# qingqing-zijin/LEAD-YOLO

Hardware: AMD Instinct MI355X
Metric: images/sec (640x640) fwd+bwd (higher is better)
Workload: dtype bf16; 1 GPU; lead-yolo-s bs=64/gpu 3x640x640 bf16 full train step: uint8 batch -> train-mode forward (batch-statistics BN), ComputeLoss, HIP backward, clip 10, SGD-nesterov 3 groups, ModelEMA update (BASELINE.json configs[2]); random-init weights; global_batch=64, parallelism=dp1 (single GPU, no collective), world_size=1

## Files before the change

### include/lead_yolo_hip.h

```cpp
#ifndef LEAD_YOLO_HIP_H
#define LEAD_YOLO_HIP_H
#ifdef __cplusplus
extern "C" {
#endif

enum { LY_F32 = 0, LY_BF16 = 1 };
int ly_abi_version(void);
const char* ly_last_error(void);

int ly_mlpblock_fwd(const void* x , void* y , int n_img, int H, int W, int C, const void* wp, const void* w1,
                    const void* w2, const float* bn_scale, const float* bn_shift, double* stats, int dtype, void* stream);
int ly_mlpblock_pconv(const void* x , void* z , int n_img, int H, int W, int C, const void* wp, int dtype, void* stream);
int ly_mlpblock_bwd_ok(int C, int dtype);
long ly_mlpblock_bwd_slab_floats(int C);
int ly_mlpblock_bwd(const void* x , const void* dy , void* g , int n_img, int H, int W, int C, const void* wp, const void* w1,
                    const void* w2t, const void* w1t, const float* a, const float* b, const float* alpha, const float* kappa, const float* lambda,
                    double* stats, float* slab, long slab_floats, float* dw1, float* dw2, int pass, int dtype, void* stream);
int ly_mlpblock_bwd_dx_ok(int C, int W, int dtype);
int ly_mlpblock_bwd_dx(const void* g , const void* dy , const void* x , void* dx , int n_img, int H, int W, int C, const void* wpt,
                       float* slab, long slab_floats, float* dwp, int lddw, int dw_ts, int dw_cs, int dtype, void* stream);
int ly_mlpblock_hidden_tiles(int C);

enum { LY_ACT_NONE_ = 0, LY_ACT_RELU_ = 1, LY_ACT_SILU_ = 2 };
enum { LY_GATHER_ROWS = 0,
       LY_GATHER_UP2 = 1,
       LY_GATHER_PATCH = 2,
       LY_GATHER_PATCH_NCHW = 3,
       LY_GATHER_PATCH_NCHW_U8 = 4,
       LY_GATHER_PATCH_NCHW_BF16 = 5,
       LY_GATHER_PATCH_NCHW_F16 = 6    };
enum { LY_PRO_NONE = 0,
       LY_PRO_GATE = 1,
       LY_PRO_AFFINE_RELU_CA = 2      };

typedef struct LyGemmParams {
  long M;
  int H, W;
  int K, N;
  const void* a0; int lda0; int k0;
  const void* a1; int lda1;
  int gather;
  int Hin, Win, Cin, ks, pk;
  int pro;
  const float* g_h; const float* g_w;
  const void* res; int ldres;
  const float* p_scale; const float* p_shift; const float* p_ca;
  const void* wp;
  const float* e_scale; const float* e_shift;
  const float* rowscale;
  int act;
  void* out; int ldo;
  double* stats;
  int dtype;
  int scat_ks, scat_c;
  const void* eadd; int ldeadd;
} LyGemmParams;

int ly_gemm_fwd(const LyGemmParams* p, void* stream);


typedef struct LyConv3Params {
  long M; int H, W;
  int Cin, N;
  int TH, TW;
  const void* x; int ldx;
  const void* wp;
  const float* e_scale; const float* e_shift;
  int act;
  void* out; int ldo;
  double* stats;
  int dtype;
} LyConv3Params;

int ly_conv3x3_fwd(const LyConv3Params* p, void* stream);


int ly_pool_hw(const void* x , int ldx, int n_img, int H, int W, int C, float* pool, int dtype, void* stream);
int ly_coordatt_mlp(const float* pool, int n_img, int H, int W, int C, int mip, const float* w1, const float* b1,
                    const float* sc, const float* sh, const float* wh, const float* bh, const float* ww, const float* bw, float* a_h,
                    float* a_w, void* stream);
int ly_coordatt_mlp_bwd(const float* pool, int n_img, int H, int W, int C, int mip, const float* w1, const float* b1,
                        const float* mean, const float* invstd, const float* gamma, const float* beta, const float* wh,
                        const float* ww, const float* a_h, const float* a_w, const float* da_h, const float* da_w, float* ws,
                        double* sums , float* dpool, float* dw1, float* dgamma, float* dbeta, float* dwh, float* dbh, float* dww,
                        float* dbw, int grads_f64 , void* stream);

int ly_coordatt_gate(const void* x , int ldx, int n_img, int H, int W, int C, const float* a_h, const float* a_w,
                     const void* res , int ldres, void* out , int ldo, int dtype, void* stream);

int ly_se_fwd(const void* x , int ldx, int n_img, int HW, int C, const float* wa, const float* wb, int R, float* part,
              int slices, float* ca, int dtype, void* stream);
int ly_rfcbam_stats(const void* x , int ldx, int n_img, int H, int W, int C, int k, int s, const float* wg,
                    const float* a1, const float* b1, int TH, int TW, float* mm, float* part, int slices, int dtype, void* stream);
int ly_colsum(const void* x , int ldx, int n_img, int HW, int C, float* part, int slices, int dtype, void* stream);
int ly_rfcbam_mid(const float* part, int slices, int C, int HW, const float* wa, const float* wb, int R, float* ca, int n_img,
                  const float* mm, int HK, int WK, const float* w18, float* rfa, void* stream);
int ly_rfa_map(const float* mm, int n_img, int HK, int WK, const float* w, float* rfa, void* stream);

typedef struct LyRfcbam3Params {
  int n_img, H, W, C;
  int Ho, Wo, N, s;
  int TH, TW;
  const void* x; int ldx;
  const float* wg;
  const float* ca;
  const float* rfa;
  const void* wp;
  const float* e_scale; const float* e_shift;
  void* out; int ldo;
  double* stats;
  int linear;
  int dtype;
} LyRfcbam3Params;
int ly_rfcbam3_fwd(const LyRfcbam3Params* p, void* stream);

int ly_rf3c_stats(const void* x , int ldx, int n_img, int H, int W, int C, int s, const float* wq, int raw, int TH, int TW, float* mm,
                  float* part, int slices, int dtype, void* stream);
int ly_rf3c_fwd(const LyRfcbam3Params* p, const float* wq, int raw, void* stream);

int ly_rf3m_stats(const void* x , int ldx, int n_img, int H, int W, int C, int s, const void* wst, int TH, int TW, float* mm, float* part,
                  int slices, void* stream);
int ly_rf3m_fwd(const LyRfcbam3Params* p, void* stream);

typedef struct LyRf3cBwdParams {
  int n_img, H, W, C;
  int Ho, Wo, O, s;
  int TH, TW;
  const void* x; int ldx;
  const void* du; int lddu;
  const float* wq;
  const void* wct;
  const float* ca;
  const float* rfa;
  const float* mm;
  const float* d_mm;
  const float* coef;
  float* d_rfa_part; float* d_ca;
  float* sums;
  float* dwg;
  void* dx; int lddx;
  const float* dgap; float dgap_scale;
  float* dwc_part; int ng;
  int dtype;
} LyRf3cBwdParams;
int ly_rf3c_bwd(const LyRf3cBwdParams* p, int pass, void* stream);
int ly_rf3c_wgrad(const LyRf3cBwdParams* p, void* stream);


int ly_sppf_pool(const void* x , int ldx, int n_img, int H, int W, int C, int k, void* out , int ldo, int dtype, void* stream);
int ly_detect_tail(const void* y , int ldy, int n_img, int H, int W, int na, int no, const float* anchors, float stride,
                   float* p, float* z, long zrows, long zoff, int dtype, void* stream);
int ly_detect_level(const void* x , int ldx, int n_img, int H, int W, int K, const void* wp, int nat, const float* bias, int na, int no,
                    const float* anchors, float stride, float* p, float* z, long zrows, long zoff, int dtype, void* stream);
int ly_detect_level_ok(int K, int na, int no, int dtype);
int ly_detect_level_aug(const void* x , int ldx, int n_img, int H, int W, int K, const void* wp, int nat, const float* bias, int na, int no,
                        const float* anchors, float stride, float* p, float* z, long zrows, long zoff, float dscale, int dflip, float img_w,
                        int dtype, void* stream);
int ly_detect_tail_aug(const void* y , int ldy, int n_img, int H, int W, int na, int no, const float* anchors, float stride,
                       float* p, float* z, long zrows, long zoff, float dscale, int dflip, float img_w, int dtype, void* stream);

enum { LY_F16 = 2 };
#define LY_SCALE_IMG_MAX 4
typedef struct LyScaleImgSpec {
  void* out;
  int Hs, Ws;
  int Ho, Wo;
  int flip;
} LyScaleImgSpec;
int ly_scale_img(const void* x , int n_img, int C, int H, int W, const LyScaleImgSpec* specs, int nspec, float pad, int dtype, void* stream);

typedef struct LyMosaicTile {
  long off;
  int h, w;
  int x1a, y1a, x2a, y2a;
  int x1b, y1b;
  int lab, nlab;
  int src;
  int unused;
  double padw, padh;
} LyMosaicTile;
typedef struct LyMosaicImage {
  LyMosaicTile tile[4];
  double m[6];
  float minv[6];
  double scale;
  int mosaic;
  int flipud, fliplr;
  int unused;
  const unsigned char* lut;
} LyMosaicImage;
int ly_mosaic_img(const unsigned char* bank, const LyMosaicImage* imgs, int n_img, int s, unsigned char* out, void* stream);
int ly_mosaic_labels(const double* labels, const LyMosaicImage* imgs, int n_img, int s, int max_labels, float* targets, long cap, void* stream);
typedef struct LyMixup {
  int partner;
  int unused;
  double r;
} LyMixup;
int ly_mosaic_mix_img(const unsigned char* bank, const LyMosaicImage* imgs, const LyMixup* mix, int n_img, int n_entry, int s, unsigned char* out,
                      void* stream);
int ly_mosaic_mix_labels(const double* labels, const LyMosaicImage* imgs, const LyMixup* mix, int n_img, int n_entry, int s, int max_labels,
                         float* targets, long cap, void* stream);
int ly_detect_head_bwd(const float* dp, int n_img, int H, int W, int na, int no, void* du , int ldu, float* dbias,
                       int dbias_f64 , int dtype, void* stream);


int ly_chan_moments(const void* x , int ldx, long rows, int C, double* mom , int dtype, void* stream);
int ly_coordatt_conv1_stats(const float* pool, long positions, int C, int mip, const float* w1, const float* b1,
                            double* stats , void* stream);
int ly_sum_rows_f64(const double* src, int R, int C, double* dst, void* stream);

int ly_rfcbam_tap_moments(const void* x , int ldx, int n_img, int H, int W, int C, int s, double* mom , int dtype, void* stream);
int ly_rfcbam_gen_prepare(const double* mom, int C, int k, const float* gen_w, const float* gamma, const float* beta, float eps,
                          float momentum, double count, float* running_mean, float* running_var, long* nbt, float* out8, float* a1,
                          float* wq_stats, float* wq_main, float* wq_c , int mom_stripes , void* stream);

int ly_nms_candidates(const float* pred, int bs, int N, int no, float conf_thres, unsigned long long class_mask, float* score, float* det,
                      void* stream);
int ly_nms_candidates_ml(const float* pred, int bs, int N, int no, float conf_thres, unsigned long long class_mask, float* score, float* det,
                         void* stream);
int ly_nms_greedy(const float* det, const long* order, const float* sorted_score, int bs, int N, float iou_thres, float max_wh, int max_det,
                  int max_nms, int* keep, int* count, void* stream);

#define LY_VAL_MAX_LABELS 512
int ly_val_match(const float* dets, const int* counts, int bs, int max_det, const float* targets, long nt, int W, int H, const float* shapes,
                 const float* levels, int single_cls, int nc, const int* cursor, int capacity, int row_width, void* correct, float* conf,
                 float* cls, int* match_label, float* match_iou, int* n_det, int* nt_class, int* overflow, void* stream);
int ly_val_advance(int* cursor, int bs, void* stream);
int ly_val_confusion(const float* dets, const int* counts, int bs, int max_det, const float* targets, long nt, int W, int H,
                     const float* shapes, float conf_thres, float iou_thres, int single_cls, int nc, int* matrix, int* flags, void* stream);

typedef struct LyLetterboxImage {
  const unsigned char* src;
  unsigned char* dst;
  int h0, w0;
  int H, W;
  int nh, nw;
  int top, left;
} LyLetterboxImage;
enum { LY_LB_CHW_RGB = 0, LY_LB_HWC_BGR = 1 };
int ly_letterbox_u8(const LyLetterboxImage* imgs, int n_img, int maxH, int maxW, int layout, void* stream);
int ly_scale_boxes(const float* dets, const int* counts, int bs, int max_det, const float* shapes, int round_boxes, float* out,
                   void* stream);


int ly_bnact_fwd(const void* u , int ldu, long rows, int C, const float* a, const float* b, int act, void* y , int ldy, int dtype, void* stream);
int ly_bnact_bwd_reduce(const void* dy , int lddy, const void* u , int ldu, long rows, int C, const float* a, const float* b,
                        int act, double* sums , int dtype, void* stream);
int ly_bnact_bwd_apply(const void* dy , int lddy, const void* u , int ldu, long rows, int C, const float* a, const float* b,
                       int act, const float* alpha, const float* kappa, const float* lambda, void* du , int lddu, int dtype, void* stream);
int ly_bnact_bwd_reduce_pair(const void* dy1 , int lddy1, const void* dy2 , int lddy2, int csplit, const void* u , int ldu, long rows, int C,
                             const float* a, const float* b, int act, double* sums1, double* sums2, int dtype, void* stream);
int ly_bnact_bwd_apply_pair(const void* dy1 , int lddy1, const void* dy2 , int lddy2, int csplit, const void* u , int ldu, long rows, int C,
                            const float* a, const float* b, int act, const float* alpha, const float* kappa, const float* lambda, void* du , int lddu,
                            int dtype, void* stream);

typedef struct LyWgradParams {
  long M;
  int H, W;
  int N;
  const void* du; int lddu;
  const void* x; int ldx;
  int Hin, Win, Cin;
  int ks, stride, pad;
  int nchw, up2;
  float* dw; int lddw;
  int dtype;
  int dw_ts, dw_cs, n_valid, c_valid;
  const float* x_scale; const float* x_shift;
  float* ws; long ws_floats;
} LyWgradParams;
int ly_wgrad(const LyWgradParams* p, void* stream);
int ly_wgrad_group(const LyWgradParams* arr, int n, void* stream);
int ly_tune_wgrad3(int on);

int ly_up2_bwd(const void* d , int ldd, int n_img, int Hs, int Ws, int C, void* out , int ldo, int dtype, void* stream);
int ly_unpatch(const void* g , int n_img, int Ho, int Wo, int C, int ks, void* dx , int dtype, void* stream);
int ly_sum_rows(const float* src, long R, long C, long ld, float* dst, int accumulate, void* stream);
int ly_patch4_rows_u8(const unsigned char* img, int n_img, int C, int H, int W, void* rows , int dtype, void* stream);
int ly_patch4_wgrad_u8(const unsigned char* img, int n_img, int C, int H, int W, const void* du , int lddu, int N, float scale, float* slab,
                       long slab_floats, float* dw , int dtype, void* stream);

int ly_coordatt_gate_bwd(const void* dout , int ldd, const void* x , int ldx, int n_img, int H, int W, int C, const float* a_h,
                         const float* a_w, void* dx , int lddx, float* da_h, float* da_w, int bands, int slabs, int dtype, void* stream);
int ly_pool_hw_bwd(const float* gp, int n_img, int H, int W, int C, void* dx , int lddx, int accumulate, int dtype, void* stream);
int ly_maxpool_arg(const void* x , int ldx, int n_img, int H, int W, int C, int k, unsigned char* arg, int lda, int dtype, void* stream);
int ly_maxpool_gather(const unsigned char* arg, int lda, const float* d_up, int ldu, const void* d_own, int ldd, int own_dtype, int n_img, int H,
                      int W, int C, int k, void* out, int ldo, int out_dtype, void* stream);
int ly_sppf_bwd(const void* buf , int ldb, const void* d , int ldd, int n_img, int H, int W, int c, int k, void* out , int ldo, int dtype,
                void* stream);
int ly_mlp_dx(const void* dy , const void* g , const void* t , int ldt, long rows, int C, int c4, void* dx , int dtype, void* stream);
int ly_maxpool_bwd(const void* x , int ldx, const float* dy, int lddy, int n_img, int H, int W, int C, int k, float* dx, int lddx,
                   int dtype, void* stream);

int ly_rf_generate(const void* x , int ldx, int n_img, int H, int W, int C, int k, int s, const float* wg, void* ug , int dtype, void* stream);
int ly_rf_bwd_attn(int n_img, int H, int W, int C, int k, int s, const void* ug , const void* dcd , const float* ag, const float* bg,
                   const float* ca, const float* rfa, void* cd , float* d_rfa, float* gmax, float* d_ca, int dtype, void* stream);
int ly_rfa_bwd(const float* d_rfa, const float* rfa, const float* mm, const float* w18, int n_img, int Hk, int Wk, float* d_mm,
               float* dw18, int dw18_f64 , void* stream);
int ly_rf_bwd_relu(int n_img, int H, int W, int C, int k, int s, const void* ug , void* dcd , const float* ag, const float* bg,
                   const float* ca, const float* rfa, const float* gmax, const float* d_mm, float* sums, int dtype, void* stream);
int ly_rf_bwd_gen(const void* x , int ldx, int n_img, int H, int W, int C, int k, int s, const void* ug , void* dv , const float* alpha,
                  const float* kappa, const float* lambda, float* dwg, int part_rows, int dtype, void* stream);
int ly_rf_bwd_dx(int n_img, int H, int W, int C, int k, int s, const void* dug , const float* wg, void* dx , int lddx,
                 const float* addnc , float add_scale,
                 int dtype, void* stream);
int ly_se_bwd(const float* part, int slices, int n_img, int HW, int C, const float* wa, const float* wb, int R, const float* ca,
              const void* d_ca , int d_ca_f64, float* dwa, float* dwb,
              float* dgap, float* ws, void* stream);

#define LY_STATS_STRIPES 32
int ly_bn_finalize(const void* stats , int stats_f64, int stripes, int nch, int c_off, int N, double count, const float* gamma, const float* beta,
                   const float* bias, float eps, float momentum, float* running_mean, float* running_var, long* nbt, float* scale,
                   float* shift, float* mean, float* invstd, void* stream);
int ly_bn_bwd_coeffs(const void* sums , int sums_f64, int stripes, int N, double count, const float* a,
                     const float* mean, const float* invstd, int train, float* dgamma, float* dbeta, float* alpha, float* kappa, float* lambda,
                     int tr_a, int tr_b , void* stream);
int ly_bn_finalize_pair(const void* stats, int stats_f64, int stripes, int c_half, double count, const float* gamma0, const float* beta0, float eps0,
                        float momentum0, float* running_mean0, float* running_var0, long* nbt0, const float* gamma1, const float* beta1, float eps1,
                        float momentum1, float* running_mean1, float* running_var1, long* nbt1, float* scale, float* shift, float* mean,
                        float* invstd, void* stream);
int ly_bn_bwd_coeffs_pair(const void* sums0, const void* sums1, int sums_f64, int stripes, int c_half, double count, const float* a, const float* mean,
                          const float* invstd, float* dgamma0, float* dbeta0, float* dgamma1, float* dbeta1, float* alpha, float* kappa,
                          float* lambda, void* stream);
int ly_frag_pack3(const float* w, int R, int K, long ld_r, long ld_k, int rows_to, int planes, void* out, void* stream);

typedef struct LyPackDesc {
  const float* src; void* dst;
  int r_valid, K, planes, S, t0, T;
  int nrb, nb, nc, vb, vc;
  long sra, srb, sa, sb, sc;
  long blk0;
} LyPackDesc;
int ly_pack_table(const LyPackDesc* table, const int* blk_desc, int n_blocks, void* stream);

typedef struct LyRf1BwdParams {
  int n_img; long HW; int C;
  const void* x; int ldx;
  const void* dcd;
  const float* gw; const float* ag; const float* bg; const float* ca; const float* rfa;
  void* cd; float* d_rfa; float* gmax_out; double* d_ca;
  const float* gmax; const float* d_mm; double* sums;
  const float* alpha; const float* kappa; const float* lambda; const float* dgap; float dgap_scale;
  void* dx; int lddx; float* dgw;
  int dtype;
  int dgw_f64;
} LyRf1BwdParams;
int ly_rf1_bwd(const LyRf1BwdParams* p, int pass, void* stream);
#define LY_F64_ADD_MAX 64
typedef struct LyF64AddTable {
  const double* src[LY_F64_ADD_MAX];
  float* dst[LY_F64_ADD_MAX];
  int n[LY_F64_ADD_MAX];
  int count;
} LyF64AddTable;
int ly_f64_add(const LyF64AddTable* t, void* stream);
int ly_rf3s_bwd(const LyRf1BwdParams* p, int Ho, int Wo, int pass, void* stream);

int ly_loss_level(const float* p, float* dp, const float* anchors, const float* targets, int bs, int na, int ny, int nx, int no, long nt,
                  float anchor_t, float box_gain, float obj_gain, float balance, float* tobj, int* winner, long* cand_cell, float* cand,
                  float* acc, float* tbox, int match_only, float cls_gain, float cp, float cn, float cls_pw, float obj_pw, void* stream);
int ly_loss_finish(const float* acc, int nl, const float* cells, const float* balance, float box_gain, float obj_gain, float cls_gain, int nc,
                   int bs, float* out, void* stream);

typedef struct LyOptTensor {
  float* p;
  float* g;
  float* buf;
  float* ema;
  long n;
  float wd;
  int group;
  int taps, cin;
} LyOptTensor;
int ly_optim_step(const LyOptTensor* table, const int* blk_tensor, const long* blk_off, int n_blocks, double* ws, float* hyper,
                  float* norm_out, void* stream);

typedef struct LyAdamTensor {
  float* p;
  float* g;
  float* m;
  float* v;
  float* ema;
  long n;
  float wd;
  int group;
  int taps, cin;
  int step0;
} LyAdamTensor;
int ly_adam_step(const LyAdamTensor* table, const int* blk_tensor, const long* blk_off, int n_blocks, double* ws, float* hyper,
                 int decoupled, float* norm_out, void* stream);

int ly_event_create(void** event);
int ly_event_destroy(void* event);
int ly_event_record(void* event, void* stream);
int ly_stream_wait_event(void* stream, void* event);

#ifdef __cplusplus
}
#endif
#endif
```

### lead-yolo_amd/csrc/ly_backward.hip

```cpp
#include "ly_tile.hpp"
#include "ly_params.h"
#include "ly_wgrad.hpp"

template <int ACT>
__device__ __forceinline__ f32x4 ly_dact4(const f32x4 v, const f32x4 dy) {
  f32x4 r;
#pragma unroll
  for (int i = 0; i < 4; ++i) {
    if (ACT == LY_ACT_RELU) {
      r[i] = v[i] > 0.f ? dy[i] : 0.f;
    } else if (ACT == LY_ACT_SILU) {
      const float s = ly_sigmoid(v[i]);
      r[i] = dy[i] * s * (1.f + v[i] * (1.f - s));
    } else {
      r[i] = dy[i];
    }
  }
  return r;
}

#ifndef LY_XCD_STREAM
#define LY_XCD_STREAM 1
#endif
#if LY_XCD_STREAM
// ... 458 lines not shown
    const int quads = t_isA[u] ? BN / 4 : BK / 4;
    const int cq = tt % quads;
    t_g[u] = (tt / quads) % PG;
    t_row[u] = (t_isA[u] ? 0 : BN) + 4 * cq;
    if (t_isA[u]) {
      t_c[u] = n0 + 4 * cq;
      t_ok[u] = live && t_c[u] < Q.N;
      t_ky[u] = t_kx[u] = 0;
    } else {
      const int col = k0 + 4 * cq;
      t_ok[u] = live && col < Ktot;
      const int cc = t_ok[u] ? col : 0;
      const int tap = cc / Q.Cin;
      t_c[u] = cc - tap * Q.Cin;
      t_ky[u] = tap / Q.ks;
      t_kx[u] = tap - t_ky[u] * Q.ks;
    }
    if (!live) t_row[u] = -1;
  }
  const int Hv = Q.up2 ? 2 * Q.Hin : Q.Hin, Wv = Q.up2 ? 2 * Q.Win : Q.Win;
  const float invW = 1.f / (float)Q.W, invH = 1.f / (float)Q.H;

  constexpr bool DEFER = SLAB == 2 && ROWS;
  long pre_p0 = 0;
  R4 pre[TPT][8];
  auto prefetch = [&](long p0) {
    pre_p0 = p0;
#pragma unroll
    for (int u = 0; u < TPT; ++u) {
      const long pf = p0 + 8 * t_g[u];
      int n_i = 0, ho = 0, wo = 0;
      if (!ROWS && !t_isA[u]) {
        const int g = (int)(pf < Q.M ? pf : Q.M - 1);
        const int row = ly_fdiv(g, Q.W, invW);
        wo = g - row * Q.W;
        n_i = ly_fdiv(row, Q.H, invH);
        ho = row - n_i * Q.H;
      }
#pragma unroll
      for (int j = 0; j < 8; ++j) {
        const long p = pf + j;
        bool ok = t_ok[u] && p < p_end;
        const T* src;
        if (t_isA[u]) {
          src = du + (ok ? p : p_begin) * Q.lddu + t_c[u];
        } else if (ROWS) {
          src = xin + (ok ? p : p_begin) * Q.ldx + t_c[u];
        } else {
          int hi = ho * Q.stride + t_ky[u] - Q.pad, wi = wo * Q.stride + t_kx[u] - Q.pad;
          ok = ok && hi >= 0 && hi < Hv && wi >= 0 && wi < Wv;
          if (Q.up2) { hi >>= 1; wi >>= 1; }
          src = xin + (ok ? (((long)n_i * Q.Hin + hi) * Q.Win + wi) * Q.ldx : 0) + t_c[u];
          if (++wo == Q.W) { wo = 0; if (++ho == Q.H) { ho = 0; ++n_i; } }
        }
        R4 v = ly_ldr4<T>(src);
        if constexpr (!DEFER) {
          if (!ok) ly_zero_raw(v);
        }
        pre[u][j] = v;
      }
    }
  };
  auto commit = [&](int buf) {
    char* base = lds + buf * BUF;
#pragma unroll
    for (int u = 0; u < TPT; ++u) {
      if (t_row[u] < 0) continue;
      if constexpr (DEFER) {
#pragma unroll
        for (int j = 0; j < 8; ++j)
          if (!(t_ok[u] && pre_p0 + 8 * t_g[u] + j < p_end)) ly_zero_raw(pre[u][j]);
      }
      const bool pb = pro && !t_isA[u];
      f32x4 sa = ly_zero4(), sh = ly_zero4();
      if constexpr (ROWS && PRO) {
        const int lc = t_isA[u] ? 0 : t_row[u] - BN;
        sa = *reinterpret_cast<const f32x4*>(sab + lc);
        sh = *reinterpret_cast<const f32x4*>(sab + BK + lc);
      }
      if constexpr (PL == 2) {
#pragma unroll
        for (int e = 0; e < 4; ++e) {
          float v[8] = {pre[u][0][e], pre[u][1][e], pre[u][2][e], pre[u][3][e], pre[u][4][e], pre[u][5][e], pre[u][6][e], pre[u][7][e]};
          if constexpr (ROWS && PRO) {
#pragma unroll
            for (int j = 0; j < 8; ++j) v[j] = pb ? fmaxf(v[j] * sa[e] + sh[e], 0.f) : v[j];
          }
          bf16x8 hi, lo;
          ly_split8(v, hi, lo);
          char* d = base + t_g[u] * PLANE + t_row[u] * 4 + e * ((NR / 4 + 4) * 16);
          *reinterpret_cast<bf16x8*>(d) = hi;
          *reinterpret_cast<bf16x8*>(d + PG * PLANE) = lo;
        }
      } else {
        bf16x4 q[8];
#pragma unroll
        for (int j = 0; j < 8; ++j) q[j] = __builtin_bit_cast(bf16x4, pre[u][j]);
        if constexpr (ROWS && PRO) {
#pragma unroll
          for (int j = 0; j < 8; ++j) {
            f32x4 v = ly_cvt4(q[j]) * sa + sh;
#pragma unroll
            for (int e = 0; e < 4; ++e) v[e] = fmaxf(v[e], 0.f);
            const bf16x4 r = ly_cvtb4(v);
            q[j] = pb ? r : q[j];
          }
        }
#pragma unroll
        for (int e = 0; e < 4; ++e) {
          const bf16x8 row = {q[0][e], q[1][e], q[2][e], q[3][e], q[4][e], q[5][e], q[6][e], q[7][e]};
          *reinterpret_cast<bf16x8*>(base + t_g[u] * PLANE + t_row[u] * 4 + e * ((NR / 4 + 4) * 16)) = row;
        }
      }
    }
  };

  bool o_isA[OC ? TPT8 : 1], o_ok[OC ? TPT8 : 1];
  int o_row[OC ? TPT8 : 1], o_g[OC ? TPT8 : 1], o_c[OC ? TPT8 : 1], o_ky[OC ? TPT8 : 1], o_kx[OC ? TPT8 : 1];
  ly_u32x4 pre8[OC ? TPT8 : 1][OC ? 8 : 1];
  if constexpr (OC) {
#pragma unroll
    for (int u = 0; u < TPT8; ++u) {
      const int t = tid + u * LY_THREADS;
      const bool live = t < TASKS8;
      o_isA[u] = t < (BN / 8) * PG;
      const int tt = o_isA[u] ? t : t - (BN / 8) * PG;
      const int octs = o_isA[u] ? BN / 8 : BK / 8;
      const int co = tt % octs;
      o_g[u] = (tt / octs) % PG;
      o_row[u] = live ? (o_isA[u] ? 0 : BN) + 8 * co : -1;
      o_c[u] = (o_isA[u] ? n0 : k0) + 8 * co;
      o_ok[u] = live && o_c[u] < (o_isA[u] ? Q.N : Ktot);
      o_ky[u] = o_kx[u] = 0;
      if (!ROWS && !o_isA[u]) {
        const int cc = o_ok[u] ? o_c[u] : 0;
        const int tap = cc / Q.Cin;
        o_c[u] = cc - tap * Q.Cin;
        o_ky[u] = tap / Q.ks;
        o_kx[u] = tap - o_ky[u] * Q.ks;
      }
    }
  }
  auto prefetch8 = [&](long p0) {
    pre_p0 = p0;
#pragma unroll
    for (int u = 0; u < (OC ? TPT8 : 0); ++u) {
      const long pf = p0 + 8 * o_g[u];
      int n_i = 0, ho = 0, wo = 0;
      if (!ROWS && !o_isA[u]) {
        const int g = (int)(pf < Q.M ? pf : Q.M - 1);
        const int row = ly_fdiv(g, Q.W, invW);
        wo = g - row * Q.W;
        n_i = ly_fdiv(row, Q.H, invH);
        ho = row - n_i * Q.H;
      }
#pragma unroll
      for (int j = 0; j < 8; ++j) {
        const long p = pf + j;
        bool ok = o_ok[u] && p < p_end;
        const T* src;
        if (o_isA[u]) {
          src = du + (ok ? p : p_begin) * Q.lddu + (ok ? o_c[u] : 0);
        } else if (ROWS) {
          src = xin + (ok ? p : p_begin) * Q.ldx + (ok ? o_c[u] : 0);
        } else {
          int hi = ho * Q.stride + o_ky[u] - Q.pad, wi = wo * Q.stride + o_kx[u] - Q.pad;
          ok = ok && hi >= 0 && hi < Hv && wi >= 0 && wi < Wv;
          if (Q.up2) { hi >>= 1; wi >>= 1; }
          src = xin + (ok ? (((long)n_i * Q.Hin + hi) * Q.Win + wi) * Q.ldx + o_c[u] : 0);
          if (++wo == Q.W) { wo = 0; if (++ho == Q.H) { ho = 0; ++n_i; } }
        }
        ly_u32x4 v = *reinterpret_cast<const ly_u32x4*>(src);
        if constexpr (!DEFER) {
          if (!ok) v = (ly_u32x4){0u, 0u, 0u, 0u};
        }
        pre8[u][j] = v;
      }
    }
  };
  auto commit8 = [&](int buf) {
    char* base = lds + buf * BUF;
#pragma unroll
    for (int u = 0; u < (OC ? TPT8 : 0); ++u) {
      if (o_row[u] < 0) continue;
      if constexpr (DEFER) {
#pragma unroll
        for (int j = 0; j < 8; ++j)
          if (!(o_ok[u] && pre_p0 + 8 * o_g[u] + j < p_end)) pre8[u][j] = (ly_u32x4){0u, 0u, 0u, 0u};
      }
      if constexpr (PRO) {
        if (pro && !o_isA[u]) {
          const int lc = o_row[u] - BN;
          const f32x4 sa0 = *reinterpret_cast<const f32x4*>(sab + lc), sa1 = *reinterpret_cast<const f32x4*>(sab + lc + 4);
          const f32x4 sh0 = *reinterpret_cast<const f32x4*>(sab + BK + lc), sh1 = *reinterpret_cast<const f32x4*>(sab + BK + lc + 4);
#pragma unroll
          for (int j = 0; j < 8; ++j) {
            f32x4 q[2];
            ly_rv_unpack(pre8[u][j], q);
            q[0] = q[0] * sa0 + sh0;
            q[1] = q[1] * sa1 + sh1;
#pragma unroll
            for (int e = 0; e < 4; ++e) { q[0][e] = fmaxf(q[0][e], 0.f); q[1][e] = fmaxf(q[1][e], 0.f); }
            pre8[u][j] = ly_rv_pack(q, (ly_u32x4*)nullptr);
          }
        }
      }
      char* const d0 = base + o_g[u] * PLANE + (o_row[u] >> 3) * 16;
#pragma unroll
      for (int e = 0; e < 8; ++e) {
        ly_u32x4 row;
#pragma unroll
        for (int k = 0; k < 4; ++k)
          row[k] = __builtin_amdgcn_perm(pre8[u][2 * k + 1][e >> 1], pre8[u][2 * k][e >> 1], (e & 1) ? 0x07060302u : 0x05040100u);
        *reinterpret_cast<ly_u32x4*>(d0 + e * ((NR / 8 + 2) * 16)) = row;
      }
    }
  };
  auto prefetch_any = [&](long p0) { if constexpr (OC) prefetch8(p0); else prefetch(p0); };
  auto commit_any = [&](int buf) { if constexpr (OC) commit8(buf); else commit(buf); };

  f32x4 acc[NI][NJ];
#pragma unroll
  for (int i = 0; i < NI; ++i)
#pragma unroll
    for (int j = 0; j < NJ; ++j) acc[i][j] = ly_zero4();
  const int wn = (wave & 1) * (BN / 2), wk = BN + (wave >> 1) * (BK / 2);
  const int rd_a = lq * PLANE + rowoff(li) + (wn / 16) * ISTEP, rd_b = lq * PLANE + rowoff(li) + (wk / 16) * ISTEP;

  prefetch_any(p_begin);
  commit_any(0);
  __syncthreads();
  int buf = 0;
  for (long p0 = p_begin; p0 < p_end; p0 += P) {
    const bool more = p0 + P < p_end;
    if (more) prefetch_any(p0 + P);
    const char* base = lds + buf * BUF;
#pragma unroll
    for (int ks = 0; ks < P / 32; ++ks) {
      bf16x8 ah[NI], al[NI];
#pragma unroll
      for (int i = 0; i < NI; ++i) {
        const char* r = base + rd_a + ks * (4 * PLANE) + i * ISTEP;
        ah[i] = *reinterpret_cast<const bf16x8*>(r);
        al[i] = PL == 2 ? *reinterpret_cast<const bf16x8*>(r + (PL - 1) * PG * PLANE) : ah[i];
      }
#pragma unroll
      for (int j = 0; j < NJ; ++j) {
        const char* r = base + rd_b + ks * (4 * PLANE) + j * ISTEP;
        const bf16x8 bh = *reinterpret_cast<const bf16x8*>(r);
        const bf16x8 bl = PL == 2 ? *reinterpret_cast<const bf16x8*>(r + (PL - 1) * PG * PLANE) : bh;
#pragma unroll
        for (int i = 0; i < NI; ++i) acc[i][j] = ly_mfmapp<PL>(ah[i], al[i], bh, bl, acc[i][j]);
      }
    }
    if constexpr (SB) {
      __syncthreads();
      if (more) commit_any(0);
      __syncthreads();
    } else {
      if (more) commit_any(buf ^ 1);
      __syncthreads();
      buf ^= 1;
    }
  }

  if (SLAB == 2 || (SLAB == 1 && slab)) {
    float* const sl = slab + ((long)chunk_idx * tiles + tile_idx) * (BN * BK);
#pragma unroll
    for (int i = 0; i < NI; ++i)
#pragma unroll
      for (int j = 0; j < NJ; ++j) {
        const int lc = (wave >> 1) * (BK / 2) + 16 * j + li;
        const int col = k0 + lc;
        if (col >= Ktot) continue;
        const int tap = col / Q.Cin, cch = col - tap * Q.Cin;
        if (cch >= Q.c_valid) continue;
#pragma unroll
        for (int r = 0; r < 4; ++r) {
          const int lr = wn + 16 * i + 4 * lq + r;
          if (n0 + lr < Q.n_valid) sl[lr * BK + lc] = acc[i][j][r];
        }
      }
    return;
  }
  if constexpr (SLAB != 2) {
#pragma unroll
  for (int i = 0; i < NI; ++i)
#pragma unroll
    for (int j = 0; j < NJ; ++j) {
      const int col = k0 + (wave >> 1) * (BK / 2) + 16 * j + li;
      if (col >= Ktot) continue;
      const int tap = col / Q.Cin, cch = col - tap * Q.Cin;
      if (cch >= Q.c_valid) continue;
      const long cidx = (long)tap * Q.dw_ts + (long)cch * Q.dw_cs;
#pragma unroll
      for (int r = 0; r < 4; ++r) {
        const int row = n0 + wn + 16 * i + 4 * lq + r;
        if (row < Q.n_valid) atomicAdd(Q.dw + (long)row * Q.lddw + cidx, acc[i][j][r]);
      }
    }
  }
}

__device__ __forceinline__ void ly_wgrad_combine_body(const LyWgradParams& P, const float* __restrict__ slab, const int chunks, const int tiles_k,
                                                      const int tiles, const int BN, const int BK, const long blk, const int rls) {
  const long E = (long)tiles * BN * BK;
  const long e = blk * 64 + (threadIdx.x & 63);
  const int tile = (int)(e / (BN * BK));
  const int rem = (int)(e - (long)tile * (BN * BK));
  const int lr = rem / BK, lc = rem - lr * BK;
  const int tk = tile % tiles_k, tn = tile / tiles_k;
  const int row = tn * BN + lr, col = tk * BK + lc;
  const int tap = col / P.Cin, cch = col - tap * P.Cin;
  const bool live = e < E && row < P.n_valid && col < P.ks * P.ks * P.Cin && cch < P.c_valid;
  ly_wgrad_fold(slab + e, E, chunks, rls, live, P.dw + (long)row * P.lddw + (long)tap * P.dw_ts + (long)cch * P.dw_cs);
}
__global__ __launch_bounds__(1024) void ly_wgrad_combine_kernel(const LyWgradParams P, const float* __restrict__ slab, const int chunks, const int tiles_k,
                                                               const int tiles, const int BN, const int BK, const int rls) {
  ly_wgrad_combine_body(P, slab, chunks, tiles_k, tiles, BN, BK, (long)blockIdx.x, rls);
}
static void wgrad_combine_launch(const LyWgradParams& P, const float* slab, long chunks, int tiles_k, long tiles, int BN, int BK, hipStream_t st) {
  const long E = tiles * BN * BK;
  const int rls = chunks <= 192 ? 4 : 16;
  hipLaunchKernelGGL(ly_wgrad_combine_kernel, dim3((unsigned)((E + 63) / 64)), dim3(64 * rls), 0, st, P, slab, (int)chunks, tiles_k, (int)tiles, BN, BK, rls);
}

template <typename T, int BN, int BK, int P, bool ROWS, bool PRO = false, bool OCT = false>
__global__ __launch_bounds__(LY_THREADS) __attribute__((amdgpu_waves_per_eu(BN + BK > 160 ? 2 : 3))) void ly_wgrad_tiled_kernel(const LyWgradParams P_, const int tiles_k, const long chunk_px, float* const slab) {
  ly_wgrad_tiled_body<T, BN, BK, P, ROWS, PRO, 1, OCT>(P_, (int)blockIdx.x, (int)blockIdx.y, tiles_k, chunk_px, slab, (int)gridDim.x);
}

#define LY_WGRAD_GROUP_MAX 4
struct LyWgradGroupArgs {
  LyWgradParams p[LY_WGRAD_GROUP_MAX];
  long chunk_px[LY_WGRAD_GROUP_MAX];
  float* slab[LY_WGRAD_GROUP_MAX];
  int tiles_k[LY_WGRAD_GROUP_MAX], tiles[LY_WGRAD_GROUP_MAX], blk0[LY_WGRAD_GROUP_MAX + 1];
  int chunks[LY_WGRAD_GROUP_MAX], cblk0[LY_WGRAD_GROUP_MAX + 1];
  int n;
};
template <typename T, int BN, int BK, int P, bool ROWS, bool PRO = false, bool GSLAB = false, bool OCT = false>
__global__ __launch_bounds__(LY_THREADS) __attribute__((amdgpu_waves_per_eu(BN + BK > 160 ? 2 : 3))) void ly_wgrad_tiled_group_kernel(const LyWgradGroupArgs G) {
  const int bid = ly_xcd_remap((int)blockIdx.x, (int)gridDim.x);
  int g = 0;
#pragma unroll
  for (int i = 1; i < LY_WGRAD_GROUP_MAX; ++i)
    if (i < G.n && bid >= G.blk0[i]) g = i;
  g = __builtin_amdgcn_readfirstlane(g);
  const int local = bid - G.blk0[g];
  const int tiles = G.tiles[g];
  ly_wgrad_tiled_body<T, BN, BK, P, ROWS, PRO, GSLAB ? 2 : 0, OCT>(G.p[g], local % tiles, local / tiles, G.tiles_k[g], G.chunk_px[g], GSLAB ? G.slab[g] : nullptr, tiles);
}
__global__ __launch_bounds__(1024) void ly_wgrad_combine_group_kernel(const LyWgradGroupArgs G, const int BN, const int BK, const int rls) {
  int g = 0;
#pragma unroll
  for (int i = 1; i < LY_WGRAD_GROUP_MAX; ++i)
    if (i < G.n && (int)blockIdx.x >= G.cblk0[i]) g = i;
  g = __builtin_amdgcn_readfirstlane(g);
  ly_wgrad_combine_body(G.p[g], G.slab[g], G.chunks[g], G.tiles_k[g], G.tiles[g], BN, BK, (long)((int)blockIdx.x - G.cblk0[g]), rls);
}

static long wg_target_blocks(bool group) {
#ifdef LY_DEVEL
  static long t[2] = {0, 0};
  if (!t[group]) {
    const char* e = getenv(group ? "LY_WG_GROUP_BLOCKS" : "LY_WG_BLOCKS");
    t[group] = e && atol(e) > 0 ? atol(e) : 512;
  }
  return t[group];
#else
  (void)group;
  return 512;
#endif
}

template <typename T>
static bool wgrad_octets(const LyWgradParams& Q) {
  if constexpr (!LyT<T>::BF) return false;
#ifdef LY_DEVEL
  static int off = -1;
  if (off < 0) { const char* e = getenv("LY_WG_NO_OCT"); off = e && atoi(e) ? 1 : 0; }
  if (off) return false;
#endif
  return (Q.N & 7) == 0 && (Q.Cin & 7) == 0 && (Q.lddu & 7) == 0 && (Q.ldx & 7) == 0 && ((uintptr_t)Q.du & 15) == 0 && ((uintptr_t)Q.x & 15) == 0;
}

template <typename T, int BN, int BK, int P>
static int launch_wgrad_tiled(const LyWgradParams& Q, bool rows, hipStream_t st) {
  const int Ktot = Q.ks * Q.ks * Q.Cin;
  const int tiles_n = (Q.N + BN - 1) / BN, tiles_k = (Ktot + BK - 1) / BK;
  const long tiles = (long)tiles_n * tiles_k;
  long chunks = (wg_target_blocks(false) + tiles - 1) / tiles;
  const long max_chunks = (Q.M + 511) / 512;
  if (chunks > max_chunks) chunks = max_chunks;
  if (chunks < 1) chunks = 1;
  long chunk_px = (Q.M + chunks - 1) / chunks;
  chunk_px = (chunk_px + P - 1) / P * P;
  chunks = (Q.M + chunk_px - 1) / chunk_px;
  LY_CHECK(chunks < 65536, "wgrad: too many pixel chunks");
  const size_t lds = (LyT<T>::PL * P >= 128 ? 1 : 2) * (size_t)LyT<T>::PL * (P / 8) * (BN + BK + 16) * 16 + 2 * BK * sizeof(float);
  const dim3 grid((unsigned)tiles, (unsigned)chunks);
  const long need = chunks * tiles * (long)(BN * BK);
  float* const slab = (chunks > 1 && Q.ws && need <= Q.ws_floats) ? Q.ws : nullptr;
#define WG_TILED(ROWS_, PRO_, OCT_) \
  ly_launch_lds<ly_wgrad_tiled_kernel<T, BN, BK, P, ROWS_, PRO_, OCT_>>(grid, dim3(LY_THREADS), lds, st, Q, tiles_k, chunk_px, slab)
  const bool pro = rows && Q.x_scale;
  const auto launch = [&]() -> int {
    if constexpr (LyT<T>::BF) {
      if (wgrad_octets<T>(Q)) return !rows ? WG_TILED(false, false, true) : pro ? WG_TILED(true, true, true) : WG_TILED(true, false, true);
    }
    return !rows ? WG_TILED(false, false, false) : pro ? WG_TILED(true, true, false) : WG_TILED(true, false, false);
  };
#undef WG_TILED
  LY_TRY(launch());
  if (slab) wgrad_combine_launch(Q, slab, chunks, tiles_k, tiles, BN, BK, st);
  LY_LAUNCH_CHECK();
  return 0;
}

template <typename T>
static int wgrad_dispatch(const LyWgradParams& P, void* stream);
static int g_ly_wgrad3 = 1;
extern "C" int ly_tune_wgrad3(int on) {
  const int was = g_ly_wgrad3;
  g_ly_wgrad3 = on;
  return was;
}

extern "C" int ly_wgrad(const LyWgradParams* p, void* stream) {
  LY_CHECK(p, "wgrad: null params");
  LY_CHECK_DTYPE(p->dtype, "wgrad");
  return p->dtype == LY_BF16 ? wgrad_dispatch<__bf16>(*p, stream) : wgrad_dispatch<float>(*p, stream);
}

template <typename T>
static bool wgrad_is_rows128(const LyWgradParams& P) {
  if (!(P.du && P.x && P.dw) || !(P.M > 0 && P.H > 0 && P.W > 0 && P.N > 64 && P.Cin > 0) || P.M >= (1L << 24) || P.M % ((long)P.H * P.W) != 0) return false;
  if (!(P.ks == 1 && P.stride == 1 && P.pad == 0 && !P.nchw && !P.up2 && P.Hin == P.H && P.Win == P.W)) return false;
  if (!(P.n_valid > 0 && P.n_valid <= P.N && P.c_valid > 0 && P.c_valid <= P.Cin && P.dw_ts > 0 && P.dw_cs > 0)) return false;
  if ((long)P.lddw < (long)(P.c_valid - 1) * P.dw_cs + 1) return false;
  return (P.N & 3) == 0 && (P.Cin & 3) == 0 && (P.lddu & 3) == 0 && (P.ldx & 3) == 0 && ((uintptr_t)P.du & (4 * sizeof(T) - 1)) == 0 &&
         ((uintptr_t)P.x & (4 * sizeof(T) - 1)) == 0;
}

template <typename T>
static int wgrad_group_launch(const LyWgradParams* arr, int n, hipStream_t st) {
  constexpr int PX = LyT<T>::BF ? 128 : 64, BN = 128, BK = 128;
  LyWgradGroupArgs G;
  long tiles_total = 0;
  for (int g = 0; g < n; ++g) {
    G.p[g] = arr[g];
    G.tiles_k[g] = (arr[g].Cin + BK - 1) / BK;
    G.tiles[g] = ((arr[g].N + BN - 1) / BN) * G.tiles_k[g];
    tiles_total += G.tiles[g];
  }
  G.n = n;
  G.blk0[0] = 0;
  for (int g = 0; g < n; ++g) {
    long chunks = (wg_target_blocks(true) + tiles_total - 1) / tiles_total;
    const long max_chunks = (arr[g].M + 511) / 512;
    if (chunks > max_chunks) chunks = max_chunks;
    if (chunks < 1) chunks = 1;
    long chunk_px = (arr[g].M + chunks - 1) / chunks;
    chunk_px = (chunk_px + PX - 1) / PX * PX;
    chunks = (arr[g].M + chunk_px - 1) / chunk_px;
    G.chunk_px[g] = chunk_px;
    G.chunks[g] = (int)chunks;
    G.blk0[g + 1] = G.blk0[g] + (int)(chunks * G.tiles[g]);
  }
  for (int g = n; g < LY_WGRAD_GROUP_MAX; ++g) { G.tiles_k[g] = G.tiles[g] = 1; G.chunk_px[g] = PX; G.blk0[g + 1] = G.blk0[n]; G.p[g] = arr[0]; G.chunks[g] = 0; G.slab[g] = nullptr; }
  bool gslab = arr[0].ws != nullptr && (long)G.blk0[n] * (BN * BK) <= arr[0].ws_floats;
  G.cblk0[0] = 0;
  for (int g = 0; g < n; ++g) {
    G.slab[g] = gslab ? arr[0].ws + (long)G.blk0[g] * (BN * BK) : nullptr;
    G.cblk0[g + 1] = G.cblk0[g] + (int)(((long)G.tiles[g] * BN * BK + 63) / 64);
  }
  for (int g = n; g < LY_WGRAD_GROUP_MAX; ++g) G.cblk0[g + 1] = G.cblk0[n];
  const size_t lds = (LyT<T>::PL * PX >= 128 ? 1 : 2) * (size_t)LyT<T>::PL * (PX / 8) * (BN + BK + 16) * 16 + 2 * BK * sizeof(float);
  bool any_pro = false;
  for (int g = 0; g < n; ++g) any_pro = any_pro || arr[g].x_scale != nullptr;
  bool oct = true;
  for (int g = 0; g < n; ++g) oct = oct && wgrad_octets<T>(arr[g]);
#define WG_GROUP(PRO_, GSLAB_, OCT_) \
  ly_launch_lds<ly_wgrad_tiled_group_kernel<T, BN, BK, PX, true, PRO_, GSLAB_, OCT_>>(dim3((unsigned)G.blk0[n]), dim3(LY_THREADS), lds, st, G)
  const auto launch = [&]() -> int {
    if (!gslab) return any_pro ? WG_GROUP(true, false, false) : WG_GROUP(false, false, false);
    if constexpr (LyT<T>::BF) {
      if (oct) return any_pro ? WG_GROUP(true, true, true) : WG_GROUP(false, true, true);
    }
    return any_pro ? WG_GROUP(true, true, false) : WG_GROUP(false, true, false);
  };
#undef WG_GROUP
  LY_TRY(launch());
  if (gslab) {
    int cmax = 0;
    for (int g = 0; g < n; ++g) cmax = G.chunks[g] > cmax ? G.chunks[g] : cmax;
    const int rls = cmax <= 64 ? 4 : 16;
    hipLaunchKernelGGL(ly_wgrad_combine_group_kernel, dim3((unsigned)G.cblk0[n]), dim3(64 * rls), 0, st, G, BN, BK, rls);
    LY_LAUNCH_CHECK();
  }
  return 0;
}

extern "C" int ly_wgrad_group(const LyWgradParams* arr, int n, void* stream) {
  LY_CHECK(arr && n > 0, "wgrad_group: bad arguments");
  bool same = n >= 2 && n <= LY_WGRAD_GROUP_MAX;
  for (int g = 0; g < n && same; ++g) {
    LY_CHECK_DTYPE(arr[g].dtype, "wgrad_group");
    same = arr[g].dtype == arr[0].dtype && (arr[g].dtype == LY_BF16 ? wgrad_is_rows128<__bf16>(arr[g]) : wgrad_is_rows128<float>(arr[g]));
  }
  if (!same) {
    for (int g = 0; g < n; ++g) {
      const int rc = ly_wgrad(arr + g, stream);
      if (rc) return rc;
    }
    return 0;
  }
  hipStream_t st = reinterpret_cast<hipStream_t>(stream);
  return arr[0].dtype == LY_BF16 ? wgrad_group_launch<__bf16>(arr, n, st) : wgrad_group_launch<float>(arr, n, st);
}

template <typename T>
static int wgrad_dispatch(const LyWgradParams& P, void* stream) {
  LY_CHECK(P.du && P.x && P.dw, "wgrad: null pointer");
  LY_CHECK(P.M > 0 && P.H > 0 && P.W > 0 && P.N > 0 && P.Cin > 0 && P.ks > 0 && P.stride > 0, "wgrad: bad sizes");
  LY_CHECK(P.M < (1L << 24), "wgrad: M=%ld pixels exceeds the 2^24 limit of the fast index path", P.M);
  LY_CHECK(P.M % ((long)P.H * P.W) == 0, "wgrad: M is not a whole number of images");
  const int Ktot = P.ks * P.ks * P.Cin;
  LY_CHECK(P.n_valid > 0 && P.n_valid <= P.N && P.c_valid > 0 && P.c_valid <= P.Cin && P.dw_ts > 0 && P.dw_cs > 0, "wgrad: bad dw layout");
  LY_CHECK((long)P.lddw >= (long)(P.ks * P.ks - 1) * P.dw_ts + (long)(P.c_valid - 1) * P.dw_cs + 1, "wgrad: lddw=%d does not cover a dw row", P.lddw);
  const bool rows = P.ks == 1 && P.stride == 1 && P.pad == 0 && !P.nchw && !P.up2;
  if (rows) LY_CHECK(P.Hin == P.H && P.Win == P.W, "wgrad: 1x1 gather needs Hin == H, Win == W");
  LY_CHECK((P.x_scale == nullptr) == (P.x_shift == nullptr), "wgrad: x_scale and x_shift come together");
  const bool tiled_ok = !P.nchw && (P.N & 3) == 0 && (P.Cin & 3) == 0 && (P.lddu & 3) == 0 && (P.ldx & 3) == 0 && ((uintptr_t)P.du & (4 * sizeof(T) - 1)) == 0 &&
                        ((uintptr_t)P.x & (4 * sizeof(T) - 1)) == 0;
  if (P.x_scale) LY_CHECK(rows && tiled_ok, "wgrad: the x prologue is built for plain-row 1x1 problems with vector-friendly widths");
  if (g_ly_wgrad3 && ly_wgrad3_ok(P)) return ly_wgrad3_launch(P, reinterpret_cast<hipStream_t>(stream));
  if (!P.nchw && (P.N & 3) == 0 && (P.Cin & 3) == 0 && (P.lddu & 3) == 0 && (P.ldx & 3) == 0 && ((uintptr_t)P.du & (4 * sizeof(T) - 1)) == 0 && ((uintptr_t)P.x & (4 * sizeof(T) - 1)) == 0) {
    hipStream_t st2 = reinterpret_cast<hipStream_t>(stream);
    constexpr int PX = LyT<T>::BF ? 128 : 64;
    if (P.N <= 64 && Ktot <= 64) return launch_wgrad_tiled<T, 64, 64, PX>(P, rows, st2);
    if (P.N <= 32) return launch_wgrad_tiled<T, 32, 128, PX>(P, rows, st2);
    if (P.N <= 64) return launch_wgrad_tiled<T, 64, 128, PX>(P, rows, st2);
    return launch_wgrad_tiled<T, 128, 128, PX>(P, rows, st2);
  }
  const int tiles_n = (P.N + 63) / 64, tiles_k = (Ktot + 63) / 64;
  const long tiles = (long)tiles_n * tiles_k;
  long chunks = (2048 + tiles - 1) / tiles;
  const long max_chunks = (P.M + 255) / 256;
  if (chunks > max_chunks) chunks = max_chunks;
  if (chunks < 1) chunks = 1;
  long chunk_px = (P.M + chunks - 1) / chunks;
  chunk_px = (chunk_px + 31) / 32 * 32;
  chunks = (P.M + chunk_px - 1) / chunk_px;
  LY_CHECK(chunks < 65536, "wgrad: too many pixel chunks");
  hipStream_t st = reinterpret_cast<hipStream_t>(stream);
  const dim3 grid((unsigned)tiles, (unsigned)chunks);
  if (rows) hipLaunchKernelGGL((ly_wgrad_kernel<T, true>), grid, dim3(LY_THREADS), 0, st, P, tiles_k, chunk_px);
  else hipLaunchKernelGGL((ly_wgrad_kernel<T, false>), grid, dim3(LY_THREADS), 0, st, P, tiles_k, chunk_px);
  LY_LAUNCH_CHECK();
  return 0;
}

template <typename T>
__global__ __launch_bounds__(LY_THREADS) void ly_up2_bwd_kernel(const T* __restrict__ d, int ldd, int n_img, int Hs, int Ws, int C,
                                                                T* __restrict__ o, int ldo) {
  const int nc4 = C >> 2;
  const long total = (long)n_img * Hs * Ws * nc4;
  for (long i = (long)blockIdx.x * LY_THREADS + threadIdx.x; i < total; i += (long)gridDim.x * LY_THREADS) {
    const long pix = i / nc4;
    const int c = 4 * (int)(i - pix * nc4);
    const long row = pix / Ws;
    const int w = (int)(pix - row * Ws);
    const long n = row / Hs;
    const int h = (int)(row - n * Hs);
    const T* s = d + (((n * 2 * Hs + 2 * h) * 2L * Ws) + 2 * w) * ldd + c;
    const f32x4 v = ly_ld4<T>(s) + ly_ld4<T>(s + ldd) + ly_ld4<T>(s + 2L * Ws * ldd) + ly_ld4<T>(s + 2L * Ws * ldd + ldd);
    ly_st4<T>(o + pix * ldo + c, v);
  }
}

extern "C" int ly_up2_bwd(const void* d, int ldd, int n_img, int Hs, int Ws, int C, void* out, int ldo, int dtype, void* stream) {
  LY_CHECK_DTYPE(dtype, "up2_bwd");
  LY_CHECK(d && out && n_img > 0 && Hs > 0 && Ws > 0 && (C & 3) == 0 && (ldd & 3) == 0 && (ldo & 3) == 0, "up2_bwd: bad arguments");
  LY_WITH_T(dtype, hipLaunchKernelGGL(ly_up2_bwd_kernel<T>, dim3((unsigned)ly_ew_blocks((long)n_img * Hs * Ws * (C >> 2))), dim3(LY_THREADS), 0,
                                      reinterpret_cast<hipStream_t>(stream), reinterpret_cast<const T*>(d), ldd, n_img, Hs, Ws, C, reinterpret_cast<T*>(out), ldo));
  LY_LAUNCH_CHECK();
  return 0;
}

template <typename T>
__global__ __launch_bounds__(LY_THREADS) void ly_unpatch_kernel(const T* __restrict__ g, int n_img, int Ho, int Wo, int C, int ks,
                                                                T* __restrict__ dx) {
  const int nc4 = C >> 2;
  const int kc = ks * ks * nc4;
  const long total = (long)n_img * Ho * Wo * kc;
  for (long i = (long)blockIdx.x * LY_THREADS + threadIdx.x; i < total; i += (long)gridDim.x * LY_THREADS) {
    const long m = i / kc;
    int r = (int)(i - m * kc);
    const int tap = r / nc4;
    const int c = 4 * (r - tap * nc4);
    const int ky = tap / ks, kx = tap - ky * ks;
    const long row = m / Wo;
    const int wo = (int)(m - row * Wo);
    const long n = row / Ho;
    const int ho = (int)(row - n * Ho);
    const long dst = ((n * Ho * ks + (long)ho * ks + ky) * ((long)Wo * ks) + (long)wo * ks + kx) * C + c;
    ly_st4<T>(dx + dst, ly_ld4<T>(g + m * ((long)ks * ks * C) + (long)tap * C + c));
  }
}

__global__ __launch_bounds__(1024) void ly_sum_rows_kernel(const float* __restrict__ src, const long R, const long C, const long ld,
                                                          float* __restrict__ dst, const int accumulate, const int rls) {
  __shared__ float red[16][64];
  const int cl = threadIdx.x & 63, rl = threadIdx.x >> 6;
  const long c = (long)blockIdx.x * 64 + cl;
  float a0 = 0.f, a1 = 0.f, a2 = 0.f, a3 = 0.f;
  if (c < C) {
    const float* p = src + c;
    long r = rl;
    for (; r + 7 * rls < R; r += 8 * rls) {
      float v[8];
#pragma unroll
      for (int k = 0; k < 8; ++k) v[k] = p[(r + rls * k) * ld];
      __builtin_amdgcn_sched_barrier(0);
      a0 += v[0]; a1 += v[1]; a2 += v[2]; a3 += v[3];
      a0 += v[4]; a1 += v[5]; a2 += v[6]; a3 += v[7];
    }
    for (; r + 3 * rls < R; r += 4 * rls) {
      float v[4];
#pragma unroll
      for (int k = 0; k < 4; ++k) v[k] = p[(r + rls * k) * ld];
      __builtin_amdgcn_sched_barrier(0);
      a0 += v[0]; a1 += v[1]; a2 += v[2]; a3 += v[3];
    }
    for (; r < R; r += rls) a0 += p[r * ld];
  }
  red[rl][cl] = (a0 + a1) + (a2 + a3);
  __syncthreads();
  if (rl == 0 && c < C) {
    float s = 0.f;
    for (int i = 0; i < rls; ++i) s += red[i][cl];
    dst[c] = accumulate ? dst[c] + s : s;
  }
}

extern "C" int ly_sum_rows(const float* src, long R, long C, long ld, float* dst, int accumulate, void* stream) {
  LY_CHECK(src && dst && R > 0 && C > 0 && ld >= C, "sum_rows: bad arguments");
  LY_CHECK((C + 63) / 64 < (1L << 31), "sum_rows: too many columns");
  const int rls = R <= 192 ? 4 : 16;
  hipLaunchKernelGGL(ly_sum_rows_kernel, dim3((unsigned)((C + 63) / 64)), dim3(64 * rls), 0, reinterpret_cast<hipStream_t>(stream), src, R, C, ld, dst,
                     accumulate, rls);
  LY_LAUNCH_CHECK();
  return 0;
}

__global__ __launch_bounds__(LY_THREADS) void ly_sum_rows_f64_kernel(const double* __restrict__ src, const int R, const int C, double* __restrict__ dst) {
  const int c = blockIdx.x * LY_THREADS + threadIdx.x;
  if (c >= C) return;
  double a = 0.0;
  for (int r = 0; r < R; ++r) a += src[(long)r * C + c];
  dst[c] = a;
}
__global__ __launch_bounds__(LY_THREADS) void ly_f64_add_kernel(const LyF64AddTable T) {
  const int e = blockIdx.y;
  const int i = blockIdx.x * LY_THREADS + threadIdx.x;
  if (e < T.count && i < T.n[e]) T.dst[e][i] += (float)T.src[e][i];
}
extern "C" int ly_f64_add(const LyF64AddTable* t, void* stream) {
  LY_CHECK(t && t->count > 0 && t->count <= LY_F64_ADD_MAX, "f64_add: bad table");
  int nmax = 0;
  for (int e = 0; e < t->count; ++e) {
    LY_CHECK(t->src[e] && t->dst[e] && t->n[e] > 0, "f64_add: entry %d is empty", e);
    nmax = t->n[e] > nmax ? t->n[e] : nmax;
  }
  hipLaunchKernelGGL(ly_f64_add_kernel, dim3((unsigned)((nmax + LY_THREADS - 1) / LY_THREADS), (unsigned)t->count), dim3(LY_THREADS), 0,
                     reinterpret_cast<hipStream_t>(stream), *t);
  LY_LAUNCH_CHECK();
  return 0;
}

extern "C" int ly_sum_rows_f64(const double* src, int R, int C, double* dst, void* stream) {
  LY_CHECK(src && dst && R > 0 && C > 0, "sum_rows_f64: bad arguments");
  hipLaunchKernelGGL(ly_sum_rows_f64_kernel, dim3((unsigned)((C + LY_THREADS - 1) / LY_THREADS)), dim3(LY_THREADS), 0, reinterpret_cast<hipStream_t>(stream), src,
                     R, C, dst);
  LY_LAUNCH_CHECK();
  return 0;
}

extern "C" int ly_unpatch(const void* g, int n_img, int Ho, int Wo, int C, int ks, void* dx, int dtype, void* stream) {
  LY_CHECK_DTYPE(dtype, "unpatch");
  LY_CHECK(g && dx && n_img > 0 && Ho > 0 && Wo > 0 && ks > 0 && (C & 3) == 0, "unpatch: bad arguments");
  LY_WITH_T(dtype, hipLaunchKernelGGL(ly_unpatch_kernel<T>, dim3((unsigned)ly_ew_blocks((long)n_img * Ho * Wo * ks * ks * (C >> 2))), dim3(LY_THREADS), 0,
                                      reinterpret_cast<hipStream_t>(stream), reinterpret_cast<const T*>(g), n_img, Ho, Wo, C, ks, reinterpret_cast<T*>(dx)));
  LY_LAUNCH_CHECK();
  return 0;
}

#define LY_P4_WO 64
template <typename T>
__global__ __launch_bounds__(LY_THREADS) void ly_patch4_rows_u8_kernel(const unsigned char* __restrict__ img, int C, int H, int W, T* __restrict__ rows) {
  extern __shared__ f32x4 ly_p4_smem[];
  T* const tile = reinterpret_cast<T*>(ly_p4_smem);
  const int Wo = W >> 2, Ho = H >> 2;
  const int K = 16 * C, KP = K + 8;
  const int wo0 = blockIdx.x * LY_P4_WO;
  const int n = blockIdx.y / Ho, ho = blockIdx.y - n * Ho;
  const int nw = Wo - wo0 < LY_P4_WO ? Wo - wo0 : LY_P4_WO;
  for (int i = threadIdx.x; i < 4 * C * LY_P4_WO; i += LY_THREADS) {
    const int wl = i & (LY_P4_WO - 1), r = i / LY_P4_WO;
    const int c = r >> 2, ky = r & 3;
    const int wc = wl < nw ? wl : nw - 1;
    const unsigned v = *reinterpret_cast<const unsigned*>(img + (((long)n * C + c) * H + 4 * ho + ky) * W + 4 * (wo0 + wc));
    T* d = tile + wl * KP + 4 * r;
    d[0] = (T)(float)(v & 255u); d[1] = (T)(float)((v >> 8) & 255u); d[2] = (T)(float)((v >> 16) & 255u); d[3] = (T)(float)(v >> 24);
  }
  __syncthreads();
  constexpr int VE = 16 / sizeof(T);
  const int vpr = K / VE;
  T* const out = rows + ((long)blockIdx.y * Wo + wo0) * K;
  for (int j = threadIdx.x; j < nw * vpr; j += LY_THREADS) {
    const int wl = j / vpr, q = j - wl * vpr;
    *reinterpret_cast<f32x4*>(out + (long)wl * K + q * VE) = *reinterpret_cast<const f32x4*>(tile + wl * KP + q * VE);
  }
}

extern "C" int ly_patch4_rows_u8(const unsigned char* img, int n_img, int C, int H, int W, void* rows, int dtype, void* stream) {
  LY_CHECK_DTYPE(dtype, "patch4_rows_u8");
  LY_CHECK(img && rows && n_img > 0 && C > 0 && C <= 16 && H > 0 && W > 0 && (H & 3) == 0 && (W & 3) == 0, "patch4_rows_u8: bad arguments");
  LY_CHECK(((uintptr_t)img & 3) == 0 && ((uintptr_t)rows & 15) == 0, "patch4_rows_u8: unaligned pointer");
  LY_CHECK((long)n_img * (H >> 2) < 65536, "patch4_rows_u8: too many patch rows");
  const dim3 grid((unsigned)(((W >> 2) + LY_P4_WO - 1) / LY_P4_WO), (unsigned)(n_img * (H >> 2)));
  LY_WITH_T(dtype, hipLaunchKernelGGL(ly_patch4_rows_u8_kernel<T>, grid, dim3(LY_THREADS), (size_t)LY_P4_WO * (16 * C + 8) * sizeof(T),
                                      reinterpret_cast<hipStream_t>(stream), img, C, H, W, reinterpret_cast<T*>(rows)));
  LY_LAUNCH_CHECK();
  return 0;
}

#define LY_CAG_RB 8
#define LY_CAG_MAXW 8
template <typename T>
__global__ __launch_bounds__(LY_THREADS) void ly_coordatt_gate_bwd_kernel(const T* __restrict__ dout, int ldd, const T* __restrict__ x,
                                                                           int ldx, int H, int W, int C, const float* __restrict__ a_h,
                                                                           const float* __restrict__ a_w, T* __restrict__ dx, int lddx,
                                                                           float* __restrict__ da_h, float* __restrict__ da_w, int bands, int slabs, long n_img) {
  __shared__ f32x4 red[LY_THREADS];
  const int nc4 = C >> 2, tid = threadIdx.x;
  const int groups = LY_THREADS / nc4;
  const int c4 = tid % nc4, g0 = tid / nc4;
  const int slab = blockIdx.x % slabs;
  const int bb = blockIdx.x / slabs;
  const long n = bb / bands;
  const int band = bb - (int)n * bands;
  const int w0 = slab * groups * LY_CAG_MAXW;
  const int h_lo = band * LY_CAG_RB, h_hi = h_lo + LY_CAG_RB < H ? h_lo + LY_CAG_RB : H;
  f32x4 accw[LY_CAG_MAXW], aw[LY_CAG_MAXW];
  bool okw[LY_CAG_MAXW];
  int wcl[LY_CAG_MAXW];
  const bool gok = g0 < groups;
#pragma unroll
  for (int i = 0; i < LY_CAG_MAXW; ++i) {
    accw[i] = ly_zero4();
    const int w = w0 + g0 + i * groups;
    okw[i] = gok && w < W;
    wcl[i] = okw[i] ? w : (w0 < W ? w0 : 0);
    aw[i] = ly_ldg4(a_w + (n * W + wcl[i]) * C + 4 * (gok ? c4 : 0));
  }
  using R4 = typename LyT<T>::R4;
  for (int h = h_lo; h < h_hi; ++h) {
    const long nh = n * H + h;
    f32x4 sh = ly_zero4();
    {
      const int c4c = gok ? c4 : 0;
      const f32x4 ah = ly_ldg4(a_h + nh * C + 4 * c4c);
      R4 dr[LY_CAG_MAXW], xr[LY_CAG_MAXW];
#pragma unroll
      for (int i = 0; i < LY_CAG_MAXW; ++i) {
        const long row = nh * W + wcl[i];
        dr[i] = ly_ldr4<T>(dout + row * ldd + 4 * c4c);
        xr[i] = ly_ldr4<T>(x + row * ldx + 4 * c4c);
      }
#pragma unroll
      for (int i = 0; i < LY_CAG_MAXW; ++i) {
        if (okw[i]) {
          const long row = nh * W + wcl[i];
          const f32x4 d = ly_r4_f32(dr[i]), xv = ly_r4_f32(xr[i]);
          ly_st4<T>(dx + row * lddx + 4 * c4, d * ah * aw[i]);
          const f32x4 t = d * xv;
          sh += t * aw[i];
          accw[i] += t * ah;
        }
      }
    }
    __syncthreads();
    red[tid] = sh;
    __syncthreads();
    if (g0 == 0) {
      for (int g = 1; g < groups; ++g) sh += red[g * nc4 + c4];
      ly_stg4(da_h + ((long)slab * n_img * H + nh) * C + 4 * c4, sh);
    }
  }
  if (g0 < groups) {
#pragma unroll
    for (int i = 0; i < LY_CAG_MAXW; ++i) {
      const int w = w0 + g0 + i * groups;
      if (w < W) {
        ly_stg4(da_w + ((long)band * n_img * W + n * W + w) * C + 4 * c4, accw[i]);
      }
    }
  }
}

extern "C" int ly_coordatt_gate_bwd(const void* dout, int ldd, const void* x, int ldx, int n_img, int H, int W, int C, const float* a_h,
                                    const float* a_w, void* dx, int lddx, float* da_h, float* da_w, int bands_in, int slabs_in, int dtype, void* stream) {
  LY_CHECK_DTYPE(dtype, "coordatt_gate_bwd");
  LY_CHECK(dout && x && a_h && a_w && dx && da_h && da_w, "coordatt_gate_bwd: null pointer");
  LY_CHECK((C & 3) == 0 && C <= 1024 && (ldd & 3) == 0 && (ldx & 3) == 0 && (lddx & 3) == 0, "coordatt_gate_bwd: C / ld must be multiples of 4");
  const int groups = LY_THREADS / (C >> 2);
  const int slabs = (W + groups * LY_CAG_MAXW - 1) / (groups * LY_CAG_MAXW);
  const int bands = (H + LY_CAG_RB - 1) / LY_CAG_RB;
  LY_CHECK(bands_in == bands && slabs_in == slabs, "coordatt_gate_bwd: the partial buffers are da_h [%d slabs][n][H][C] and da_w [%d bands][n][W][C] (got %d, %d)",
           slabs, bands, slabs_in, bands_in);
  LY_WITH_T(dtype, hipLaunchKernelGGL(ly_coordatt_gate_bwd_kernel<T>, dim3((unsigned)(n_img * bands * slabs)), dim3(LY_THREADS), 0, reinterpret_cast<hipStream_t>(stream),
                                      reinterpret_cast<const T*>(dout), ldd, reinterpret_cast<const T*>(x), ldx, H, W, C, a_h, a_w, reinterpret_cast<T*>(dx), lddx, da_h, da_w,
                                      bands, slabs, (long)n_img));
  LY_LAUNCH_CHECK();
  return 0;
}

template <typename T, bool ACC>
__global__ __launch_bounds__(LY_THREADS) void ly_pool_hw_bwd_kernel(const float* __restrict__ gp, int n_img, int H, int W, int C,
                                                                    T* __restrict__ dx, int lddx) {
  constexpr int VW = LyT<T>::VW, NQ = VW / 4;
  using RV = typename LyT<T>::RV;
  if ((C % VW) == 0 && (lddx % VW) == 0 && C / VW <= LY_THREADS) {
    const int ncv = C / VW, groups = LY_THREADS / ncv;
    const int cv = threadIdx.x % ncv, wl = threadIdx.x / ncv;
    if (wl >= groups) return;
    const int c = VW * cv;
    const float iw = 1.f / (float)W, ih = 1.f / (float)H;
    const long rows = (long)n_img * H;
    for (long nh = blockIdx.x; nh < rows; nh += gridDim.x) {
      const long n = nh / H;
      const int h = (int)(nh - n * H);
      const float* const ga = gp + (n * (H + W) + h) * C + c;
      const float* const gb = gp + (n * (H + W) + H) * C + c;
      f32x4 a[NQ];
#pragma unroll
// ... 637 lines not shown
```

### lead-yolo_amd/csrc/ly_wgrad.hpp

```cpp
#pragma once
#include "ly_common.hpp"
#include "ly_params.h"

bool ly_wgrad3_ok(const LyWgradParams& P);
int ly_wgrad3_launch(const LyWgradParams& P, hipStream_t st);

__device__ __forceinline__ void ly_wgrad_fold(const float* __restrict__ p, const long E, const int chunks, const int rls, const bool live, float* const d) {
  __shared__ float red[16 * 64];
  const int rl = threadIdx.x >> 6;
  float a0 = 0.f, a1 = 0.f, a2 = 0.f, a3 = 0.f;
  if (live) {
    int c = rl;
    for (; c + 7 * rls < chunks; c += 8 * rls) {
      float v[8];
#pragma unroll
      for (int k = 0; k < 8; ++k) v[k] = p[(long)(c + rls * k) * E];
      __builtin_amdgcn_sched_barrier(0);
      a0 += v[0]; a1 += v[1]; a2 += v[2]; a3 += v[3];
      a0 += v[4]; a1 += v[5]; a2 += v[6]; a3 += v[7];
    }
    for (; c + 3 * rls < chunks; c += 4 * rls) {
      float v[4];
#pragma unroll
      for (int k = 0; k < 4; ++k) v[k] = p[(long)(c + rls * k) * E];
      __builtin_amdgcn_sched_barrier(0);
      a0 += v[0]; a1 += v[1]; a2 += v[2]; a3 += v[3];
    }
    if (c < chunks) a0 += p[(long)c * E];
    if (c + rls < chunks) a1 += p[(long)(c + rls) * E];
    if (c + 2 * rls < chunks) a2 += p[(long)(c + 2 * rls) * E];
  }
  red[threadIdx.x] = (a0 + a1) + (a2 + a3);
  __syncthreads();
  if (rl == 0 && live) {
    float s = 0.f;
    for (int i = 0; i < rls; ++i) s += red[64 * i + threadIdx.x];
    *d += s;
  }
}
```

### lead-yolo_amd/csrc/ly_wgrad3.hip

```cpp
#include "ly_tile.hpp"
#include "ly_params.h"
#include "ly_wgrad.hpp"
#include <stdlib.h>

#define W3_BN 64
#define W3_CK 32
#define W3_RSA 160
#define W3_RSX 96
#define W3_DU_BYTES (64 * W3_RSA)
#define W3_X_BYTES (100 * W3_RSX)

typedef short w3_s16x4 __attribute__((ext_vector_type(4)));
__device__ __forceinline__ bf16x4 w3_tr(const char* p) {
  typedef __attribute__((address_space(3))) w3_s16x4 lds_s16x4;
  return __builtin_bit_cast(bf16x4, __builtin_amdgcn_ds_read_tr16_b64_v4i16((lds_s16x4*)p));
}

__global__ __launch_bounds__(LY_THREADS) __attribute__((amdgpu_waves_per_eu(4))) void ly_wgrad3_kernel(const LyWgradParams P, const int tiles_x,
                                                                                                        const int tiles_y, const int n_n,
                                                                                                        const int n_c, const int tchunk,
                                                                                                        const int total_tiles, float* __restrict__ const slab) {
  __shared__ __attribute__((aligned(16))) char w3_lds[W3_DU_BYTES + W3_X_BYTES];
  char* const ds = w3_lds;
  char* const xs = w3_lds + W3_DU_BYTES;
  const int tid = threadIdx.x, lane = tid & 63;
  const int wave = __builtin_amdgcn_readfirstlane(tid >> 6);
  const int li = lane & 15, lq = lane >> 4;
  int b = ly_xcd_remap((int)blockIdx.x, (int)gridDim.x);
  const int cn = b % n_n; b /= n_n;
  const int cc = b % n_c;
  const int chunk = b / n_c;
  const int n0 = cn * W3_BN, c0 = cc * W3_CK;
  const int t_begin = chunk * tchunk;
  const int t_end = t_begin + tchunk < total_tiles ? t_begin + tchunk : total_tiles;
  if (t_begin >= t_end) return;
  const __bf16* const du = reinterpret_cast<const __bf16*>(P.du);
  const __bf16* const x = reinterpret_cast<const __bf16*>(P.x);
  const int H = P.H, W = P.W;
  const int tiles_img = tiles_x * tiles_y;

  const int dpc = tid & 7, dpx = tid >> 3;
  const bool d_ok = n0 + 8 * dpc < P.N;
  const int xpc = tid & 3;
  const int xp0 = tid >> 2, xp1 = 64 + (tid >> 2);
  const int hy0 = xp0 / 10, hx0 = xp0 - hy0 * 10;
  const int hy1 = xp1 / 10, hx1 = xp1 - hy1 * 10;
  const bool x_ok = c0 + 8 * xpc < P.Cin;
  const bool x1_live = xp1 < 100;
  struct Regs {
    ly_u32x4 d[2], x[2];
    bool okd[2], okx[2];
  };
  Regs R0;
  auto prefetch = [&](Regs& R, int tile) {
    const int n = tile / tiles_img;
    const int r = tile - n * tiles_img;
    const int tyi = r / tiles_x, txi = r - tyi * tiles_x;
    const int oy0 = tyi * 8, ox0 = txi * 8;
#pragma unroll
    for (int e = 0; e < 2; ++e) {
      const int slot = dpx + 32 * e;
      const int oy = oy0 + (slot >> 3), ox = ox0 + (slot & 7);
      R.okd[e] = d_ok && oy < H && ox < W;
      const long off = R.okd[e] ? (((long)n * H + oy) * W + ox) * P.lddu + n0 + 8 * dpc : 0;
      R.d[e] = *reinterpret_cast<const ly_u32x4*>(du + off);
    }
#pragma unroll
    for (int e = 0; e < 2; ++e) {
      const int iy = oy0 - 1 + (e ? hy1 : hy0), ix = ox0 - 1 + (e ? hx1 : hx0);
      R.okx[e] = x_ok && (e == 0 || x1_live) && iy >= 0 && iy < H && ix >= 0 && ix < W;
      const long off = R.okx[e] ? (((long)n * H + iy) * W + ix) * P.ldx + c0 + 8 * xpc : 0;
      R.x[e] = *reinterpret_cast<const ly_u32x4*>(x + off);
    }
  };
  auto commit = [&](const Regs& R) {
    const ly_u32x4 z = {0u, 0u, 0u, 0u};
#pragma unroll
    for (int e = 0; e < 2; ++e) *reinterpret_cast<ly_u32x4*>(ds + (dpx + 32 * e) * W3_RSA + 16 * dpc) = R.okd[e] ? R.d[e] : z;
    *reinterpret_cast<ly_u32x4*>(xs + xp0 * W3_RSX + 16 * xpc) = R.okx[0] ? R.x[0] : z;
    if (x1_live) *reinterpret_cast<ly_u32x4*>(xs + xp1 * W3_RSX + 16 * xpc) = R.okx[1] ? R.x[1] : z;
  };

  const int wn = wave & 1, wk = wave >> 1;
  const int r0 = 4 * lq + (li >> 2);
  const int chunk8 = (li & 3) * 8;
  const char* a_base = ds + r0 * W3_RSA + (wn * 32) * 2 + chunk8;
  int hb[2][2];
#pragma unroll
  for (int ks = 0; ks < 2; ++ks)
#pragma unroll
    for (int e = 0; e < 2; ++e) {
      const int t = ks * 32 + 16 * e + r0;
      hb[ks][e] = ((t >> 3) * 10 + (t & 7)) * W3_RSX + chunk8;
    }
  int coff[9];
#pragma unroll
  for (int j = 0; j < 9; ++j) {
    const int ct = 9 * wk + j;
    const int tap = ct >> 1;
    const int ky = tap / 3, kx = tap - 3 * ky;
    coff[j] = (ky * 10 + kx) * W3_RSX + (ct & 1) * 32;
  }

  f32x4 acc[2][9];
#pragma unroll
  for (int i = 0; i < 2; ++i)
#pragma unroll
    for (int j = 0; j < 9; ++j) acc[i][j] = ly_zero4();

  auto contract = [&]() {
#pragma unroll
    for (int ks = 0; ks < 2; ++ks) {
      bf16x8 af[2];
#pragma unroll
      for (int i = 0; i < 2; ++i) {
        const char* p = a_base + (ks * 32) * W3_RSA + i * 32;
        af[i] = ly_cat8(w3_tr(p), w3_tr(p + 16 * W3_RSA));
      }
#pragma unroll
      for (int j = 0; j < 9; ++j) {
        const bf16x8 bf = ly_cat8(w3_tr(xs + hb[ks][0] + coff[j]), w3_tr(xs + hb[ks][1] + coff[j]));
#pragma unroll
        for (int i = 0; i < 2; ++i) acc[i][j] = ly_mfma_bf16(af[i], bf, acc[i][j]);
      }
    }
  };
  prefetch(R0, t_begin);
  for (int tile = t_begin; tile < t_end; ++tile) {
    __syncthreads();
    commit(R0);
    prefetch(R0, tile + 1 < t_end ? tile + 1 : tile);
    __syncthreads();
    contract();
  }

  if (slab) {
    float* const sl = slab + ((long)(chunk * n_c + cc) * n_n + cn) * (W3_BN * 288);
#pragma unroll
    for (int j = 0; j < 9; ++j) {
      const int ct = 9 * wk + j;
      if (c0 + (ct & 1) * 16 + li >= P.c_valid) continue;
#pragma unroll
      for (int i = 0; i < 2; ++i)
#pragma unroll
        for (int r = 0; r < 4; ++r) {
          const int row = wn * 32 + 16 * i + 4 * lq + r;
          if (n0 + row < P.n_valid) sl[row * 288 + 16 * ct + li] = acc[i][j][r];
        }
    }
    return;
  }
#pragma unroll
  for (int j = 0; j < 9; ++j) {
    const int ct = 9 * wk + j;
    const int tap = ct >> 1;
    const int cch = c0 + (ct & 1) * 16 + li;
    if (cch >= P.c_valid) continue;
    const long cidx = (long)tap * P.dw_ts + (long)cch * P.dw_cs;
#pragma unroll
    for (int i = 0; i < 2; ++i)
#pragma unroll
      for (int r = 0; r < 4; ++r) {
        const int row = n0 + wn * 32 + 16 * i + 4 * lq + r;
        if (row < P.n_valid) atomicAdd(P.dw + (long)row * P.lddw + cidx, acc[i][j][r]);
      }
  }
}

__global__ __launch_bounds__(1024) void ly_wgrad3_combine_kernel(const LyWgradParams P, const float* __restrict__ slab, const int chunks, const int n_n,
                                                                const int n_c, const int rls) {
  const long E = (long)n_c * n_n * (W3_BN * 288);
  const long e = (long)blockIdx.x * 64 + (threadIdx.x & 63);
  const int combo = (int)(e / (W3_BN * 288));
  const int rem = (int)(e - (long)combo * (W3_BN * 288));
  const int row = rem / 288, col = rem - row * 288;
  const int cn = combo % n_n, cc = combo / n_n;
  const int ct = col >> 4, li = col & 15;
  const int orow = cn * W3_BN + row;
  const int cch = cc * W3_CK + (ct & 1) * 16 + li;
  const bool live = e < E && orow < P.n_valid && cch < P.c_valid;
  ly_wgrad_fold(slab + e, E, chunks, rls, live, P.dw + (long)orow * P.lddw + (long)(ct >> 1) * P.dw_ts + (long)cch * P.dw_cs);
}

bool ly_wgrad3_ok(const LyWgradParams& P) {
  return P.dtype == LY_BF16 && P.ks == 3 && P.stride == 1 && P.pad == 1 && !P.nchw && !P.up2 && P.Hin == P.H && P.Win == P.W &&
         (P.N & 7) == 0 && (P.Cin & 7) == 0 && (P.lddu & 7) == 0 && (P.ldx & 7) == 0 && (reinterpret_cast<uintptr_t>(P.du) & 15) == 0 &&
         (reinterpret_cast<uintptr_t>(P.x) & 15) == 0;
}

int ly_wgrad3_launch(const LyWgradParams& P, hipStream_t st) {
  const int tiles_x = (P.W + 7) / 8, tiles_y = (P.H + 7) / 8;
  const long n_img = P.M / ((long)P.H * P.W);
  const long total = n_img * tiles_x * tiles_y;
  LY_CHECK(total < (1L << 30), "wgrad3: too many tiles");
  const int n_n = (P.N + W3_BN - 1) / W3_BN, n_c = (P.Cin + W3_CK - 1) / W3_CK;
#ifdef LY_DEVEL
  static int target = 0;
  if (!target) { const char* e = getenv("LY_W3_BLOCKS"); target = e ? atoi(e) : 768; }
  static const bool force_atomic = getenv("LY_W3_ATOMIC") != nullptr;
#else
  constexpr int target = 768;
  constexpr bool force_atomic = false;
#endif
  long chunks = (target + (long)n_n * n_c - 1) / ((long)n_n * n_c);
  if (chunks > total) chunks = total;
  if (chunks < 1) chunks = 1;
  const long tchunk = (total + chunks - 1) / chunks;
  chunks = (total + tchunk - 1) / tchunk;
  const long need = chunks * n_n * n_c * (long)(W3_BN * 288);
  float* slab = (P.ws && need <= P.ws_floats && !force_atomic) ? P.ws : nullptr;
  hipLaunchKernelGGL(ly_wgrad3_kernel, dim3((unsigned)(chunks * n_n * n_c)), dim3(LY_THREADS), 0, st, P, tiles_x, tiles_y, n_n, n_c, (int)tchunk,
                     (int)total, slab);
  if (slab) {
    const long E = (long)n_n * n_c * (W3_BN * 288);
    const int rls = chunks <= 192 ? 4 : 16;
    hipLaunchKernelGGL(ly_wgrad3_combine_kernel, dim3((unsigned)((E + 63) / 64)), dim3(64 * rls), 0, st, P, slab, (int)chunks, n_n, n_c, rls);
  }
  LY_LAUNCH_CHECK();
  return 0;
}
```

### lead-yolo_amd/ops.py

```python
import ctypes
import os

import torch

from . import capi
from .capi import (ACT_NONE, ACT_RELU, ACT_SILU, GATHER_PATCH, GATHER_PATCH_NCHW, GATHER_PATCH_NCHW_BF16, GATHER_PATCH_NCHW_F16, GATHER_PATCH_NCHW_U8, GATHER_ROWS, GATHER_UP2,
                   PRO_AFFINE_RELU_CA, PRO_GATE, PRO_NONE)


PROFILE = None


class _Timed:

    def __init__(self, name, flops, nbytes, valu_flops=0.0):
        self.rec = None
        if PROFILE is not None:
            self.rec = [name, float(flops), float(nbytes), torch.cuda.Event(enable_timing=True), torch.cuda.Event(enable_timing=True), float(valu_flops)]

    def __enter__(self):
        if self.rec is not None:
            self.rec[3].record()

    def __exit__(self, *a):
# ... 300 lines not shown
def se_attention(x, ldx, n, hw, c, wa, wb, r, want_part=False):
    slices = se_slices(hw)
    part = torch.empty((n, slices, c), dtype=torch.float32, device=x.device)
    ca = torch.empty((n, c), dtype=torch.float32, device=x.device)
    with _Timed(f"ly_colsum_kernel<{_tname(x)}> + ly_se_mlp_kernel", 1.0 * n * hw * c, x.element_size() * n * hw * c):
        capi.check(capi.lib().ly_se_fwd(_p(x), ldx, n, hw, c, _p(wa), _p(wb), r, _p(part), slices, _p(ca), capi.dtype_code(x), capi.stream_ptr()),
                   "ly_se_fwd")
    return (ca, part) if want_part else ca


def se_bwd(part, n, hw, c, wa, wb, r, ca, d_ca, dwa, dwb):
    if d_ca.dtype not in (torch.float32, torch.float64) or d_ca.numel() != n * c or not d_ca.is_contiguous():
        raise ValueError("se_bwd: d_ca must be a contiguous float32 / float64 [n, c]")
    dgap = torch.empty((n, c), dtype=torch.float32, device=part.device)
    ws = torch.empty(n * (2 * c + 2 * r), dtype=torch.float32, device=part.device)
    capi.check(capi.lib().ly_se_bwd(_p(part), part.shape[1], n, hw, c, _p(wa), _p(wb), r, _p(ca), _p(d_ca), int(d_ca.dtype == torch.float64), _p(dwa), _p(dwb), _p(dgap), _p(ws),
                                    capi.stream_ptr()), "ly_se_bwd")
    return dgap


def se_slices(hw):
    return max(1, min(hw // 64, 128))


def colsum(x, ldx, n, hw, c):
    slices = se_slices(hw)
    part = torch.empty((n, slices, c), dtype=torch.float32, device=x.device)
    with _Timed(f"ly_colsum_kernel<{_tname(x)}>", 1.0 * n * hw * c, x.element_size() * n * hw * c):
        capi.check(capi.lib().ly_colsum(_p(x), ldx, n, hw, c, _p(part), slices, capi.dtype_code(x), capi.stream_ptr()), "ly_colsum")
    return part


def pick_tile(ho, wo):
    best = None
    for nct in range(1, 9):
        tw = -(-wo // nct)
        if tw > 64:
            continue
        th = max(1, 64 // tw)
        th = min(th, ho)
        nrt = -(-ho // th)
        eff = (ho * wo) / (nct * nrt * 64.0)
        if best is None or eff > best[0] + 1e-9:
            best = (eff, th, tw)
    if best is None:
        return 1, 64
    return best[1], best[2]


def rf3c_ok(c, s):
    return c % 32 == 0 and s in (1, 2)


RF3M_MIN_UNITS = 1500


CONCURRENT_PARTS = 1


def rf3m_ok(x, c, o, s, n=None, ho=None, wo=None):
    if not ((x if isinstance(x, torch.dtype) else x.dtype) == torch.bfloat16 and c % 32 == 0 and o % 64 == 0 and s in (1, 2)):
        return False
    if n is None:
        return True
    th, tw = pick_tile_m(ho, wo, s)
    return n * CONCURRENT_PARTS * -(-ho // th) * -(-wo // tw) * (o // (128 if o % 128 == 0 else 64)) >= RF3M_MIN_UNITS


def pick_tile_m(ho, wo, s):
    best = None
    for tw in range(1, 33):
        for th in range(1, 32 // tw + 1):
            pos = (s * (th - 1) + 3) * (s * (tw - 1) + 3)
            if pos > 160 or th > ho or tw > max(wo, 1) * 2:
                continue
            key = (-(-ho // th) * -(-wo // tw), pos)
            if best is None or key < best[0]:
                best = (key, th, tw)
    return best[1], best[2]


def rf3m_stats(x, ldx, n, h, w, c, s, wst, th, tw, gap=True):
    ho, wo = (h + 2 - 3) // s + 1, (w + 2 - 3) // s + 1
    mm = torch.empty((n, 3 * ho, 3 * wo, 2), dtype=torch.float32, device=x.device)
    tiles = -(-ho // th) * -(-wo // tw)
    part = torch.empty((n, tiles, c), dtype=torch.float32, device=x.device) if gap else None
    with _Timed("ly_rf3m_stats_kernel", 2.0 * n * ho * wo * (c // 4) * 6 * 32 * 16, x.element_size() * n * h * w * c + 4.0 * 18 * n * ho * wo):
        capi.check(capi.lib().ly_rf3m_stats(_p(x), ldx, n, h, w, c, s, _p(wst), th, tw, _p(mm), _p(part), tiles, capi.stream_ptr()), "ly_rf3m_stats")
    return mm, part


def rf3m_fwd(*, n, h, w, c, ho, wo, N, s, th, tw, x, ldx, ca, rfa, wp, e_scale, e_shift, out, ldo):
    P = capi.LyRfcbam3Params(n, h, w, c, ho, wo, N, s, th, tw, _p(x), ldx, None, _p(ca), _p(rfa), _p(wp), _p(e_scale),
                             _p(e_shift), _p(out), ldo, None, 0, capi.dtype_code(x))
    mo = n * ho * wo
    mt = 4 if N % 128 == 0 else 2
    with _Timed(f"ly_rf3m_fwd_kernel<{mt}>", 2.0 * mo * 9 * c * N + 2.0 * mo * (N // (32 * mt)) * (c // 4) * 6 * 32 * 16,
                x.element_size() * (n * h * w * c + mo * N) + 2.0 * 9 * c * N):
        capi.check(capi.lib().ly_rf3m_fwd(ctypes.byref(P), capi.stream_ptr()), "ly_rf3m_fwd")


def pick_tile_c(ho, wo, s):
    best = None
    for tw in range(2, 65, 2):
        th = min(64 // tw, ho)
        if th < 1:
            continue
        pos = (s * (th - 1) + 3) * (s * (tw - 1) + 3)
        if pos > 320:
            continue
        tiles = -(-ho // th) * -(-wo // tw)
        key = (tiles, pos)
        if best is None or key < best[0]:
            best = (key, th, tw)
    return best[1], best[2]


def pick_tile_bwd_dx(ho, wo, o):
    best = None
    for tw in range(2, 65, 2):
        th = min(64 // tw, ho)
        ih, iw = 2 * (th - 1) + 3, 2 * (tw - 1) + 3
        pos = ih * iw
        nct = -(-wo // tw)
        lds = 2 * pos * 128 + 288 * 128 + 64 * (2 * o + 16) + 32 * 9 * 8 * 4 + 256 + (ih + 2 * tw * nct + 2 + 27) * 128
        if th < 1 or pos > 320 or lds > 160 * 1024:
            continue
        its = sum(-(-(((th + 1 - ry) // 2) * ((tw // 2 + 1 - rx) // 2)) // 8) for ry in (0, 1) for rx in (0, 1))
        key = (-(-ho // th) * nct * its, pos)
        if best is None or key < best[0]:
            best = (key, th, tw)
    return best[1], best[2]


def rf3c_stats(x, ldx, n, h, w, c, s, wq, th, tw, gap=True, raw=False):
    ho, wo = (h + 2 - 3) // s + 1, (w + 2 - 3) // s + 1
    mm = torch.empty((n, 3 * ho, 3 * wo, 2), dtype=torch.float32, device=x.device)
    tiles = -(-ho // th) * -(-wo // tw)
    part = torch.empty((n, tiles, c), dtype=torch.float32, device=x.device) if gap else None
    with _Timed(f"ly_rf3c_stats_kernel<{_tname(x)}, {s}, {'true' if raw else 'false'}>", 0.0, x.element_size() * n * h * w * c + 4.0 * 18 * n * ho * wo, valu_flops=2.0 * n * ho * wo * c * 81):
        capi.check(capi.lib().ly_rf3c_stats(_p(x), ldx, n, h, w, c, s, _p(wq), int(raw), th, tw, _p(mm), _p(part), tiles, capi.dtype_code(x),
                                            capi.stream_ptr()), "ly_rf3c_stats")
    return mm, part


def rf3c_fwd(*, n, h, w, c, ho, wo, N, s, th, tw, x, ldx, wq, ca, rfa, wp, e_scale, e_shift, out, ldo, stats=None, linear=False, raw=False):
    P = capi.LyRfcbam3Params(n, h, w, c, ho, wo, N, s, th, tw, _p(x), ldx, None, _p(ca), _p(rfa), _p(wp), _p(e_scale),
                             _p(e_shift), _p(out), ldo, _p(stats), int(linear), capi.dtype_code(x))
    mo = n * ho * wo
    bf = x.dtype == torch.bfloat16
    cfg = "2, 8" if (N > 128 and bf) else ("2, 4" if N > 64 else "1, 4")
    with _Timed(f"ly_rf3c_fwd_kernel<{_tname(x)}, {cfg}, {s}, {'true' if raw else 'false'}>", 2.0 * mo * 9 * c * N,
                x.element_size() * (n * h * w * c + mo * N) + 4.0 * 9 * c * N, valu_flops=2.0 * mo * 81 * c):
        capi.check(capi.lib().ly_rf3c_fwd(ctypes.byref(P), _p(wq), int(raw), capi.stream_ptr()), "ly_rf3c_fwd")


PRE1_PIXELS = 64


def rfcbam_stats(x, ldx, n, h, w, c, k, s, wg=None, a1=None, b1=None, th=1, tw=64, gap=False):
    ho, wo = ((h + 2 * (k // 2) - k) // s + 1, (w + 2 * (k // 2) - k) // s + 1)
    mm = torch.empty((n, k * ho, k * wo, 2), dtype=torch.float32, device=x.device)
    part, slices = None, 0
    if gap:
        if k == 3:
            raise NotImplementedError("the fused statistics + pooling pass is built for k = 1 (for k = 3 the extra per-chunk LDS pass cost more "
                                      "than the separate ly_colsum launch it saved: measured 44 -> 69 us)")
        slices = max(1, min(h * w // PRE1_PIXELS, 128))
        part = torch.empty((n, slices, c), dtype=torch.float32, device=x.device)
    with _Timed((f"ly_rfcbam_pre1_kernel<{_tname(x)}>" if (gap and k == 1) else f"ly_rfcbam_stats{k}_kernel<{_tname(x)}>"), 0.0,
                x.element_size() * n * h * w * c + 4.0 * 2 * k * k * n * ho * wo, valu_flops=2.0 * n * ho * wo * c * (81 if k == 3 else 1)):
        capi.check(capi.lib().ly_rfcbam_stats(_p(x), ldx, n, h, w, c, k, s, _p(wg), _p(a1), _p(b1), th, tw, _p(mm), _p(part), slices,
                                              capi.dtype_code(x), capi.stream_ptr()), "ly_rfcbam_stats")
    return (mm, part) if gap else mm


def rfcbam_mid(part, hw, wa, wb, r, mm, w18):
    n, slices, c = part.shape
    _, hk, wk, _ = mm.shape
    ca = torch.empty((n, c), dtype=torch.float32, device=part.device)
    rfa = torch.empty((n, hk, wk), dtype=torch.float32, device=mm.device)
    with _Timed("ly_rfcbam_mid_kernel", 36.0 * n * hk * wk, 12.0 * n * hk * wk + 4.0 * n * slices * c):
        capi.check(capi.lib().ly_rfcbam_mid(_p(part), slices, c, hw, _p(wa), _p(wb), r, _p(ca), n, _p(mm), hk, wk, _p(w18), _p(rfa), capi.stream_ptr()),
                   "ly_rfcbam_mid")
    return ca, rfa


def rfa_map(mm, w18):
    n, hk, wk, _ = mm.shape
    rfa = torch.empty((n, hk, wk), dtype=torch.float32, device=mm.device)
    with _Timed("ly_rfa_map_kernel", 36.0 * n * hk * wk, 12.0 * n * hk * wk):
        capi.check(capi.lib().ly_rfa_map(_p(mm), n, hk, wk, _p(w18), _p(rfa), capi.stream_ptr()), "ly_rfa_map")
    return rfa


def rfcbam3(*, n, h, w, c, ho, wo, N, s, th, tw, x, ldx, wg, ca, rfa, wp, e_scale, e_shift, out, ldo, stats=None, linear=False):
    P = capi.LyRfcbam3Params(n, h, w, c, ho, wo, N, s, th, tw, _p(x), ldx, _p(wg), _p(ca), _p(rfa), _p(wp), _p(e_scale),
                             _p(e_shift), _p(out), ldo, _p(stats), int(linear), capi.dtype_code(x))
    mt = 4 if N > 128 else (2 if N > 64 else 1)
    mo = n * ho * wo
    sw = mt == 4 and n * -(-ho // th) * -(-wo // tw) * -(-N // 256) > 256
    with _Timed(f"ly_rfcbam3{'_sw' if sw else ''}_kernel<{_tname(x)}, {mt}>", 2.0 * mo * 9 * c * N,
                x.element_size() * (n * h * w * c + mo * N) + 4.0 * 9 * c * N, valu_flops=2.0 * mo * 81 * c):
        capi.check(capi.lib().ly_rfcbam3_fwd(ctypes.byref(P), capi.stream_ptr()), "ly_rfcbam3_fwd")


def sppf_pool_fits(h, w):
    return 2 * h * w * 4 * 4 <= 160 * 1024


def sppf_pool(x, ldx, n, h, w, c, k, out, ldo):
    with _Timed(f"ly_sppf_pool_kernel<{_tname(x)}>", 0.0, 5.0 * x.element_size() * n * h * w * c):
        capi.check(capi.lib().ly_sppf_pool(_p(x), ldx, n, h, w, c, k, _p(out), ldo, capi.dtype_code(x), capi.stream_ptr()), "ly_sppf_pool")


def detect_tail(y, ldy, n, h, w, na, no, anchors, stride, p, z, zrows, zoff):
    capi.check(capi.lib().ly_detect_tail(_p(y), ldy, n, h, w, na, no, _p(anchors), float(stride), _p(p), _p(z), zrows, zoff,
                                         capi.dtype_code(y), capi.stream_ptr()), "ly_detect_tail")


def detect_level_ok(k, na, no, dtype):
    return dtype in (torch.float32, torch.bfloat16) and bool(capi.lib().ly_detect_level_ok(k, na, no, capi.dtype_code(dtype)))


FUSED_DETECT_LEVEL = True


def detect_level_rows(x, cin, na, no):
    if not FUSED_DETECT_LEVEL or not detect_level_ok(cin, na, no, x.dtype):
        return None
    t, ld = rows(x)
    return (t, ld) if ld % vw_of(t) == 0 and t.data_ptr() % 16 == 0 else None


def detect_level(x, ldx, n, h, w, k, wp, bias, na, no, anchors, stride, p, z, zrows, zoff, nat=True):
    es = x.element_size()
    with _Timed(f"ly_detect_level_kernel<{_tname(x)}, {k // 32}>", 2.0 * n * h * w * k * 32, es * n * h * w * k + 8.0 * n * h * w * na * no):
        capi.check(capi.lib().ly_detect_level(_p(x), ldx, n, h, w, k, _p(wp), int(nat), _p(bias), na, no, _p(anchors), float(stride), _p(p), _p(z), zrows, zoff,
                                              capi.dtype_code(x), capi.stream_ptr()), "ly_detect_level")


def detect_tail_aug(y, ldy, n, h, w, na, no, anchors, stride, z, zrows, zoff, dscale, dflip, img_w):
    capi.check(capi.lib().ly_detect_tail_aug(_p(y), ldy, n, h, w, na, no, _p(anchors), float(stride), None, _p(z), zrows, zoff, float(dscale),
                                             int(dflip), float(img_w), capi.dtype_code(y), capi.stream_ptr()), "ly_detect_tail_aug")


def detect_level_aug(x, ldx, n, h, w, k, wp, bias, na, no, anchors, stride, z, zrows, zoff, dscale, dflip, img_w, nat=True):
    es = x.element_size()
    with _Timed(f"ly_detect_level_kernel<{_tname(x)}, {k // 32}>", 2.0 * n * h * w * k * 32, es * n * h * w * k + 4.0 * n * h * w * na * no):
        capi.check(capi.lib().ly_detect_level_aug(_p(x), ldx, n, h, w, k, _p(wp), int(nat), _p(bias), na, no, _p(anchors), float(stride), None, _p(z),
                                                  zrows, zoff, float(dscale), int(dflip), float(img_w), capi.dtype_code(x), capi.stream_ptr()),
                   "ly_detect_level_aug")


SCALE_IMG_PAD = 0.447
_IMG_DTYPES = {torch.float32: capi.LY_F32, torch.bfloat16: capi.LY_BF16, torch.float16: capi.LY_F16}


def scale_img(x, specs, pad=SCALE_IMG_PAD):
    if not x.is_cuda:
        raise RuntimeError(f"scale_img: the HIP path needs a CUDA/ROCm tensor (got {x.device}); there is no CPU fallback")
    if x.dtype not in _IMG_DTYPES or x.dim() != 4:
        raise TypeError(f"scale_img: a float32 / bfloat16 / float16 NCHW image batch expected (got {x.dtype}, {tuple(x.shape)})")
    if not 1 <= len(specs) <= capi.SCALE_IMG_MAX:
        raise ValueError(f"scale_img: 1..{capi.SCALE_IMG_MAX} outputs per launch (got {len(specs)})")
    x = x.contiguous()
    n, c, h, w = x.shape
    outs = [torch.empty((n, c, ho, wo), dtype=x.dtype, device=x.device) for (_, _, ho, wo, _) in specs]
    arr = (capi.LyScaleImgSpec * len(specs))(*[capi.LyScaleImgSpec(o.data_ptr(), hs, ws, ho, wo, int(bool(fl)))
                                               for o, (hs, ws, ho, wo, fl) in zip(outs, specs)])
    tn = {torch.float32: "float", torch.bfloat16: "__bf16", torch.float16: "_Float16"}[x.dtype]
    with _Timed(f"ly_scale_img_kernel<{tn}>", 0.0, x.element_size() * sum(n * c * (h * w + ho * wo) for (_, _, ho, wo, _) in specs)):
        capi.check(capi.lib().ly_scale_img(_p(x), n, c, h, w, arr, len(specs), float(pad), _IMG_DTYPES[x.dtype], capi.stream_ptr()), "ly_scale_img")
    return outs


def detect_head_bwd(dp, n, h, w, na, no, du, ldu, dbias):
    capi.check(capi.lib().ly_detect_head_bwd(_p(dp), n, h, w, na, no, _p(du), ldu, _p(dbias), int(dbias.dtype == torch.float64), capi.dtype_code(du),
                                             capi.stream_ptr()), "ly_detect_head_bwd")


class _SmallGrads:
    pending = []
    task = -1
    announced = set()
    nodes = {}


DETERMINISTIC_SMALL_GRADS = True


def _graph_task():
    task = getattr(torch._C, "_current_graph_task_id", None)
    return task() if task is not None else -1


def small_grads_ok():
    return DETERMINISTIC_SMALL_GRADS and _graph_task() != -1


def small_grads_reset():
    _SmallGrads.pending, _SmallGrads.task, _SmallGrads.announced, _SmallGrads.nodes = [], -1, set(), {}
    _WgradQueue.items, _WgradQueue.notify, _WgradQueue.task = [], [], -1


def small_grad_scratch(target, param):
    task = _graph_task()
    if task != _SmallGrads.task:
        _SmallGrads.pending, _SmallGrads.task, _SmallGrads.announced, _SmallGrads.nodes = [], task, set(), {}
        torch.autograd.Variable._execution_engine.queue_callback(flush_small_grads)
    tgt = target.view(-1)
    for scr, t, prm in _SmallGrads.pending:
        if t.data_ptr() == tgt.data_ptr() and t.numel() == tgt.numel():
            return scr
    node = _autograd_node()
    if GRAD_LISTENERS and SMALL_GRADS_EARLY_FLUSH and node is not None:
        if param is not None and id(param) in _SmallGrads.announced:
            raise RuntimeError("small_grad_scratch: a parameter whose deferred gradient was already announced to the gradient listeners "
                               "receives another contribution in the same backward pass (shared weights under a GradReducer): set "
                               "ops.SMALL_GRADS_EARLY_FLUSH = False")
        old = [e for e in _SmallGrads.pending if _SmallGrads.nodes.get(id(e[0])) != node]
        if len(old) >= SMALL_GRADS_FLUSH_MIN:
            _SmallGrads.pending = [e for e in _SmallGrads.pending if _SmallGrads.nodes.get(id(e[0])) == node]
            _flush_small_items(old)
    scr = zeros_f64(target.numel(), target.device)
    if param is not None and not any(prm is param for _, _, prm in _SmallGrads.pending):
        for fn in GRAD_DEFER_LISTENERS:
            fn(param)
    _SmallGrads.pending.append((scr, tgt, param))
    _SmallGrads.nodes[id(scr)] = node
    return scr


SMALL_GRADS_EARLY_FLUSH = True
SMALL_GRADS_FLUSH_MIN = 6


def _autograd_node():
    fn = getattr(torch._C, "_current_autograd_node", None)
    n = fn() if fn is not None else None
    return id(n) if n is not None else None


def f64_round(scratches, shapes):
    assert 0 < len(scratches) <= capi.F64_ADD_MAX
    sizes = [s_.numel() for s_ in scratches]
    flat = torch.zeros(sum(sizes), dtype=torch.float32, device=scratches[0].device)
    t = capi.LyF64AddTable()
    outs, off = [], 0
    for j, (scr, n, shp) in enumerate(zip(scratches, sizes, shapes)):
        t.src[j], t.dst[j], t.n[j] = scr.data_ptr(), flat.data_ptr() + 4 * off, n
        outs.append(flat[off:off + n].view(shp))
        off += n
    t.count = len(scratches)
    capi.check(capi.lib().ly_f64_add(ctypes.byref(t), capi.stream_ptr()), "ly_f64_add")
    return outs


def flush_small_grads():
    items, _SmallGrads.pending, _SmallGrads.task = _SmallGrads.pending, [], -1
    _flush_small_items(items)
    _SmallGrads.announced, _SmallGrads.nodes = set(), {}


def _flush_small_items(items):
    for i in range(0, len(items), capi.F64_ADD_MAX):
        chunk = items[i:i + capi.F64_ADD_MAX]
        t = capi.LyF64AddTable()
        for j, (scr, tgt, _) in enumerate(chunk):
            t.src[j], t.dst[j], t.n[j] = scr.data_ptr(), tgt.data_ptr(), tgt.numel()
        t.count = len(chunk)
        capi.check(capi.lib().ly_f64_add(ctypes.byref(t), capi.stream_ptr()), "ly_f64_add")
    done = set()
    for _, _, prm in items:
        if prm is not None and id(prm) not in done:
            done.add(id(prm))
            _SmallGrads.announced.add(id(prm))
            grad_done(prm)


class SmallGrad:

    def __init__(self, param, numel):
        t = grad_target(param)
        self.param = param
        self.target = t = t if t is not None and t.is_contiguous() and t.numel() == numel else None
        self.deferred = t is not None and small_grads_ok()
        self.f64 = self.deferred or (t is None and DETERMINISTIC_SMALL_GRADS)
        self.buf = small_grad_scratch(t, param) if self.deferred else t.view(-1) if t is not None else \
            zeros_f64(numel, param.device) if self.f64 else torch.zeros(numel, dtype=torch.float32, device=param.device)

    def finish(self):
        if self.target is None:
            return f64_round([self.buf], [self.param.shape])[0] if self.f64 else self.buf.view(self.param.shape)
        if not self.deferred:
            grad_done(self.param)
        return None


def mlpblock(x, y, n, h, w, c, wp, w1, w2, sc, sh, stats=None):
    m = n * h * w
    cc, nt, ht, t2d = mlp_config(c, m, w, x.dtype == torch.bfloat16)
    kind = "_ring" if c >= 80 else "_occ4" if (c <= 24 and t2d == "true") else ""
    name = f"ly_mlpblock_fwd{kind}_kernel<{_tname(x)}, {cc}, {nt}, {ht}, {t2d}, {'true' if stats is not None else 'false'}>"
    if c == 80 and x.dtype == torch.bfloat16 and m >= 128 * 256 and (256 + 2 * w + 2) * 5 <= 2048:
        name = f"ly_mlpblock_res_kernel<__bf16, 80, 2, 2, {'true' if stats is not None else 'false'}, 4>"
    elif c < 80 and w % 16 == 0 and w >= 32 and n * -(-h // 8) * (w // 16) >= 1024 and (x.dtype == torch.bfloat16 or c < 40):
        name = f"ly_mlpblock_persist_kernel<{_tname(x)}, {c}, 2, {ht}, {1 if stats is not None else 0}, 1>"
    with _Timed(name, 2.0 * m * (9 * (c // 4) ** 2 + 4 * c * c),
                x.element_size() * (1 if stats is not None else 2) * m * c + 4.0 * (9 * (c // 4) ** 2 + 4 * c * c)):
        capi.check(capi.lib().ly_mlpblock_fwd(_p(x), _p(y), n, h, w, c, _p(wp), _p(w1), _p(w2), _p(sc), _p(sh), _p(stats), capi.dtype_code(x),
                                              capi.stream_ptr()), "ly_mlpblock_fwd")


def mlpblock_bwd_ok(x, c):
    return MLP_BWD_FUSED and x.dtype == torch.bfloat16 and bool(capi.lib().ly_mlpblock_bwd_ok(c, capi.dtype_code(x)))


MLP_BWD_FUSED = True


def _mlpblock_bwd_slab(c, device):
    return torch.empty(int(capi.lib().ly_mlpblock_bwd_slab_floats(c)), dtype=torch.float32, device=device)


def mlpblock_bwd(x, dy, n, h, w, c, wp, w1, w2t, w1t, a, b, *, stats=None, g=None, alpha=None, kappa=None, lam=None, dw1=None, dw2=None):
    m = n * h * w
    p1 = stats is not None
    slab = None if p1 else _mlpblock_bwd_slab(c, x.device)
    hid = 2 * c
    flops = 2.0 * m * (9 * (c // 4) ** 2 + (2 if p1 else 5) * c * hid)
    with _Timed(f"ly_mlpblock_bwd_kernel<{c}, pass {1 if p1 else 2}>", flops, x.element_size() * (2 if p1 else 3) * m * c + 4.0 * (9 * (c // 4) ** 2 + 2 * c * hid)):
        capi.check(capi.lib().ly_mlpblock_bwd(_p(x), _p(dy), _p(g), n, h, w, c, _p(wp), _p(w1), _p(w2t), _p(w1t), _p(a), _p(b), _p(alpha), _p(kappa), _p(lam),
                                              _p(stats), _p(slab), slab.numel() if slab is not None else 0, _p(dw1), _p(dw2), 1 if p1 else 2,
                                              capi.dtype_code(x), capi.stream_ptr()), "ly_mlpblock_bwd")


def mlpblock_bwd_dx_ok(x, c, w):
    return MLP_BWD_FUSED and x.dtype == torch.bfloat16 and bool(capi.lib().ly_mlpblock_bwd_dx_ok(c, w, capi.dtype_code(x)))


def mlpblock_bwd_dx(g, dy, x, n, h, w, c, wpt, dwp=None, lddw=0, dw_ts=0, dw_cs=0):
    dx = torch.empty_like(dy)
    m = n * h * w
    slab = _mlpblock_bwd_slab(c, x.device) if (dwp is not None and capi.lib().ly_mlpblock_bwd_slab_floats(c) > 0) else None
    with _Timed(f"ly_mlpblock_bwd_dx_kernel<{c}>", 2.0 * m * 18 * (c // 4) ** 2, x.element_size() * m * (3 * c + c // 4) + 4.0 * 9 * (c // 4) ** 2):
        rc = capi.lib().ly_mlpblock_bwd_dx(_p(g), _p(dy), _p(x), _p(dx), n, h, w, c, _p(wpt), _p(slab), slab.numel() if slab is not None else 0,
                                           _p(dwp if slab is not None else None), lddw, dw_ts, dw_cs, capi.dtype_code(x), capi.stream_ptr())
    if rc < 0:
        capi.check(rc, "ly_mlpblock_bwd_dx")
    return dx, rc == 0


def chan_moments(x, ldx, rows, c, f64=False, striped=False):
    mom = new_stats(c, x.device)
    with _Timed(f"ly_chan_moments_kernel<{_tname(x)}>", 3.0 * rows * c, x.element_size() * rows * c):
        capi.check(capi.lib().ly_chan_moments(_p(x), ldx, rows, c, _p(mom), capi.dtype_code(x), capi.stream_ptr()), "ly_chan_moments")
    if striped:
        return mom
    out = torch.empty(2 * c, dtype=torch.float64, device=x.device)
    capi.check(capi.lib().ly_sum_rows_f64(_p(mom), mom.shape[0], 2 * c, _p(out), capi.stream_ptr()), "ly_sum_rows_f64")
    return out if f64 else out.float()


STRIPES = capi.STATS_STRIPES


class _StatsPool:
    buf = None
    off = 0
    used = 0
    need = 0
    active = False


_POOL = _StatsPool()


def stats_pool_begin(device):
    small_grads_reset()
    p = _POOL
    if p.buf is None or p.buf.device != device or p.buf.numel() < p.need:
        p.buf = torch.zeros(max(p.need, 1), dtype=torch.float32, device=device) if p.need else None
    elif p.buf is not None:
        p.buf.zero_()
    p.off = p.used = 0
    p.active = True


def stats_pool_end():
    p = _POOL
    p.active = False
    p.need = max(p.need, p.used)


_ONES = {}


def ones_f32(numel, device):
    t = _ONES.get((numel, device))
    if t is None:
        if torch.cuda.is_current_stream_capturing():
            return torch.ones(numel, dtype=torch.float32, device=device)
        t = _ONES[(numel, device)] = torch.ones(numel, dtype=torch.float32, device=device)
    return t


def zeros_f64(numel, device):
    return zeros_f32(2 * numel, device).view(torch.float64)


def new_stats(nch, device):
    return zeros_f64(STRIPES * 2 * nch, device).view(STRIPES, 2 * nch)


def zeros_f32(numel, device):
    p = _POOL
    if p.active:
        span = (numel + 63) // 64 * 64
        p.used += span
        if p.buf is not None and p.buf.device == device and p.off + span <= p.buf.numel():
            v = p.buf[p.off:p.off + numel]
            p.off += span
            return v
    return torch.zeros(numel, dtype=torch.float32, device=device)


def bn_finalize(bn, stats, nch, count, n=None, c_off=0, pad_to=0, want_stats=False, into=None):
    n = nch if n is None else n
    dev = stats.device
    size = max(n, pad_to)
    if into is not None:
        scale, shift, mean, invstd = into
        want_stats = True
    else:
        if size > n:
            scale, shift = zeros_f32(size, dev), zeros_f32(size, dev)
        else:
            scale, shift = torch.empty(size, dtype=torch.float32, device=dev), torch.empty(size, dtype=torch.float32, device=dev)
        mean = torch.empty(n, dtype=torch.float32, device=dev) if want_stats else None
        invstd = torch.empty(n, dtype=torch.float32, device=dev) if want_stats else None
    track = bn.track_running_stats and bn.running_mean is not None
    if bn.weight is not None and bn.weight.dtype != torch.float32:
        raise NotImplementedError("train-mode BatchNorm needs float32 parameters and buffers: train under torch.autocast (fp32 master "
                                  "weights, as the reference does), not with a .half()/.bfloat16() model")
    if track and bn.momentum is None:
        raise NotImplementedError("BatchNorm with momentum=None (cumulative average) is not built")
    if track:
        from . import pack
        pack.touch()
    if stats.dtype not in (torch.float32, torch.float64):
        raise TypeError("bn_finalize: statistics must be float32 or float64")
    capi.check(capi.lib().ly_bn_finalize(_p(stats), int(stats.dtype == torch.float64), stats.shape[0], nch, c_off, n, float(count), _p(bn.weight), _p(bn.bias), None, float(bn.eps),
                                         float(bn.momentum or 0.0), _p(bn.running_mean if track else None), _p(bn.running_var if track else None),
                                         _p(bn.num_batches_tracked if track else None), _p(scale), _p(shift), _p(mean), _p(invstd),
                                         capi.stream_ptr()), "ly_bn_finalize")
    return (scale, shift, mean, invstd) if want_stats else (scale, shift)


def _bn_train_args(bn):
    track = bn.track_running_stats and bn.running_mean is not None
    if bn.weight is not None and bn.weight.dtype != torch.float32:
        raise NotImplementedError("train-mode BatchNorm needs float32 parameters and buffers: train under torch.autocast (fp32 master "
                                  "weights, as the reference does), not with a .half()/.bfloat16() model")
    if track and bn.momentum is None:
        raise NotImplementedError("BatchNorm with momentum=None (cumulative average) is not built")
    if track:
        from . import pack
        pack.touch()
    return (_p(bn.weight), _p(bn.bias), float(bn.eps), float(bn.momentum or 0.0), _p(bn.running_mean if track else None),
            _p(bn.running_var if track else None), _p(bn.num_batches_tracked if track else None))


def bn_finalize_pair(bn1, bn2, stats, c_half, count, v):
    if stats.dtype not in (torch.float32, torch.float64) or v.dtype != torch.float32 or not v.is_contiguous() or tuple(v.shape) != (4, 2 * c_half):
        raise TypeError("bn_finalize_pair: float32 / float64 statistics and a contiguous float32 [4, 2 c_half] result expected")
    capi.check(capi.lib().ly_bn_finalize_pair(_p(stats), int(stats.dtype == torch.float64), stats.shape[0], c_half, float(count), *_bn_train_args(bn1),
                                              *_bn_train_args(bn2), _p(v[0]), _p(v[1]), _p(v[2]), _p(v[3]), capi.stream_ptr()), "ly_bn_finalize_pair")


def bn_bwd_coeffs_pair(sums0, sums1, c_half, count, v, targets, coef):
    if sums0.dtype != sums1.dtype or sums0.shape != sums1.shape or sums0.dim() != 2:
        raise TypeError("bn_bwd_coeffs_pair: two striped sum arrays of one shape expected")
    (g0, b0), (g1, b1) = targets
    capi.check(capi.lib().ly_bn_bwd_coeffs_pair(_p(sums0), _p(sums1), int(sums0.dtype == torch.float64), sums0.shape[0], c_half, float(count), _p(v[0]), _p(v[2]),
                                                _p(v[3]), _p(g0), _p(b0), _p(g1), _p(b1), _p(coef[0]), _p(coef[1]), _p(coef[2]), capi.stream_ptr()),
               "ly_bn_bwd_coeffs_pair")


def bn_bwd_coeffs(sums, n, count, a, mean, invstd, train, dgamma=None, dbeta=None, transpose=None, into=None):
    dev = sums.device
    stripes = sums.shape[0] if sums.dim() == 2 else 1
    out = torch.empty(5 if into is None else 2, n, dtype=torch.float32, device=dev)
    direct = dgamma is not None and dbeta is not None
    if not direct:
        out[:2].zero_()
    capi.check(capi.lib().ly_bn_bwd_coeffs(_p(sums), int(sums.dtype == torch.float64), stripes, n, float(count), _p(a), _p(mean), _p(invstd), int(train), _p(dgamma if direct else out[0]),
                                           _p(dbeta if direct else out[1]), *[_p(t) for t in (into if into is not None else (out[2], out[3], out[4]))],
                                           *((transpose if direct else None) or (0, 0)), capi.stream_ptr()), "ly_bn_bwd_coeffs")
    al, ka, la = into if into is not None else (out[2], out[3], out[4])
    return (None if direct else out[0]), (None if direct else out[1]), al, ka, la


class GradSink:

    def __init__(self):
        self.targets = {}
        self.writes = 0

    def is_target(self, t):
        if getattr(self, "_ptr_src", None) is not self.targets or len(self.targets) != self._nptr:
            self._ptrs, self._nptr, self._ptr_src = {v.data_ptr() for v in self.targets.values()}, len(self.targets), self.targets
        return t.data_ptr() in self._ptrs

    def target(self, p):
        if p is None or not torch.is_tensor(p) or not p.requires_grad:
            return None
        t = self.targets.get(id(p))
        if t is not None and p.grad is not t:
            return None
        if t is not None:
            self.writes += 1
        return t



SINK = None
GRAD_DEFER_LISTENERS = []
GRAD_LISTENERS = []


def grad_target(p):
    return SINK.target(p) if SINK is not None else None


def grad_done(p):
    if GRAD_LISTENERS and _WgradQueue.items and SINK is not None:
        t = SINK.targets.get(id(p))
        if t is not None and any(lo <= t.data_ptr() < hi for lo, hi in map(_wgrad_span, _WgradQueue.items)):
            if all(prm is not p for prm, _ in _WgradQueue.notify):
                _WgradQueue.notify.append((p, t.data_ptr()))
                for fn in GRAD_DEFER_LISTENERS:
                    fn(p)
            return
    for fn in GRAD_LISTENERS:
        fn(p)


def coordatt_conv1_stats(pool, positions, c, mip, w1, b1):
    st = zeros_f64(2 * mip, pool.device)
    capi.check(capi.lib().ly_coordatt_conv1_stats(_p(pool), positions, c, mip, _p(w1), _p(b1), _p(st), capi.stream_ptr()),
               "ly_coordatt_conv1_stats")
    return st


def rfcbam_gen_prepare(x, ldx, n, h, w, c, k, s, gen_w, bn):
    kk = k * k
    dev = x.device
    if k == 3:
        mom = zeros_f64(54 * c, dev)
        with _Timed(f"ly_rfcbam_tap_moments_kernel<{_tname(x)}>", 108.0 * n * h * w * c / (s * s), x.element_size() * n * h * w * c):
            capi.check(capi.lib().ly_rfcbam_tap_moments(_p(x), ldx, n, h, w, c, s, _p(mom), capi.dtype_code(x), capi.stream_ptr()), "ly_rfcbam_tap_moments")
        ho, wo = (h + 2 - 3) // s + 1, (w + 2 - 3) // s + 1
        count = n * ho * wo
    else:
        mom = chan_moments(x, ldx, n * h * w, c, striped=True)
        count = n * h * w
    g = c * kk
    out8 = torch.empty(8, g, dtype=torch.float32, device=dev)
    a1 = torch.empty(c, dtype=torch.float32, device=dev) if k == 1 else None
    cps, cpm = (c + 31) // 32 * 32, (c + 15) // 16 * 16
    wqs = torch.empty(cps * 90, dtype=torch.float32, device=dev) if k == 3 else None
    wqm = torch.empty(cpm * 90, dtype=torch.float32, device=dev) if k == 3 else None
    wqc = torch.empty(c * 100, dtype=torch.float32, device=dev) if (k == 3 and c % 32 == 0) else None
    if bn.weight.dtype != torch.float32:
        raise NotImplementedError("train-mode BatchNorm needs float32 parameters and buffers")
    track = bn.track_running_stats and bn.running_mean is not None
    capi.check(capi.lib().ly_rfcbam_gen_prepare(_p(mom), c, k, _p(gen_w.detach()), _p(bn.weight.detach()), _p(bn.bias.detach()), float(bn.eps),
                                                float(bn.momentum or 0.0), float(count), _p(bn.running_mean if track else None),
                                                _p(bn.running_var if track else None), _p(bn.num_batches_tracked if track else None), _p(out8),
                                                _p(a1), _p(wqs), _p(wqm), _p(wqc), mom.shape[0] if k == 1 else 1, capi.stream_ptr()), "ly_rfcbam_gen_prepare")
    from . import pack
    pack.touch()
    return dict(gs=out8[0], gb=out8[1], gmean=out8[2], ginv=out8[3], ag=out8[4], bg=out8[5], gmean_tc=out8[6], ginv_tc=out8[7], a1=a1,
                wq_stats=wqs, wq_main=wqm, wq_c=wqc)


def bnact_fwd(u, ldu, rows, c, a, b, act, y, ldy):
    with _Timed(f"ly_bnact_fwd_kernel<{_tname(u)}, {act}>", 4.0 * rows * c, 2.0 * u.element_size() * rows * c):
        capi.check(capi.lib().ly_bnact_fwd(_p(u), ldu, rows, c, _p(a), _p(b), act, _p(y), ldy, capi.dtype_code(u), capi.stream_ptr()), "ly_bnact_fwd")


def bnact_bwd_reduce(dy, lddy, u, ldu, rows, c, a, b, act):
    sums = new_stats(c, u.device)
    with _Timed(f"ly_bnact_bwd_reduce_kernel<{_tname(u)}, {act}>", 6.0 * rows * c, 2.0 * u.element_size() * rows * c):
        capi.check(capi.lib().ly_bnact_bwd_reduce(_p(dy), lddy, _p(u), ldu, rows, c, _p(a), _p(b), act, _p(sums), capi.dtype_code(u),
                                                  capi.stream_ptr()), "ly_bnact_bwd_reduce")
    return sums


def bnact_bwd_apply(dy, lddy, u, ldu, rows, c, a, b, act, alpha, kappa, lam, du, lddu):
    with _Timed(f"ly_bnact_bwd_apply_kernel<{_tname(u)}, {act}>", 8.0 * rows * c, 3.0 * u.element_size() * rows * c):
        capi.check(capi.lib().ly_bnact_bwd_apply(_p(dy), lddy, _p(u), ldu, rows, c, _p(a), _p(b), act, _p(alpha), _p(kappa), _p(lam),
                                                 _p(du), lddu, capi.dtype_code(u), capi.stream_ptr()), "ly_bnact_bwd_apply")


def bnact_bwd_reduce_pair(dy1, lddy1, dy2, lddy2, csplit, u, ldu, rows, c, a, b, act):
    s1, s2 = new_stats(csplit, u.device), new_stats(c - csplit, u.device)
    with _Timed(f"ly_bnact_bwd_reduce_kernel<{_tname(u)}, {act}>", 6.0 * rows * c, 2.0 * u.element_size() * rows * c):
        capi.check(capi.lib().ly_bnact_bwd_reduce_pair(_p(dy1), lddy1, _p(dy2), lddy2, csplit, _p(u), ldu, rows, c, _p(a), _p(b), act, _p(s1), _p(s2),
                                                       capi.dtype_code(u), capi.stream_ptr()), "ly_bnact_bwd_reduce_pair")
    return s1, s2


def bnact_bwd_apply_pair(dy1, lddy1, dy2, lddy2, csplit, u, ldu, rows, c, a, b, act, alpha, kappa, lam, du, lddu):
    with _Timed(f"ly_bnact_bwd_apply_kernel<{_tname(u)}, {act}>", 8.0 * rows * c, 3.0 * u.element_size() * rows * c):
        capi.check(capi.lib().ly_bnact_bwd_apply_pair(_p(dy1), lddy1, _p(dy2), lddy2, csplit, _p(u), ldu, rows, c, _p(a), _p(b), act, _p(alpha), _p(kappa),
                                                      _p(lam), _p(du), lddu, capi.dtype_code(u), capi.stream_ptr()), "ly_bnact_bwd_apply_pair")


def wgrad(*, M, H, W, N, du, lddu, x, ldx, Hin, Win, Cin, dw, lddw, ks=1, stride=1, pad=0, nchw=False, up2=False, du_off=0, x_off=0,
          dw_off=0, dw_ts=None, dw_cs=1, n_valid=None, c_valid=None, x_scale=None, x_shift=None, _now=False):
    q = dict(M=M, H=H, W=W, N=N, du=du, lddu=lddu, x=x, ldx=ldx, Hin=Hin, Win=Win, Cin=Cin, dw=dw, lddw=lddw, ks=ks, stride=stride,
             pad=pad, nchw=nchw, up2=up2, du_off=du_off, x_off=x_off, dw_off=dw_off, dw_ts=dw_ts, dw_cs=dw_cs, n_valid=n_valid,
             c_valid=c_valid, x_scale=x_scale, x_shift=x_shift)
    if not _now and _wgrad_deferrable(q):
        return _wgrad_enqueue(q)
    P = _wgrad_params(**q)
    with _Timed(wgrad_kernel_name(_tname(x), N, ks * ks * Cin, ks == 1 and stride == 1 and pad == 0 and not nchw and not up2,
                                  (not nchw) and N % 4 == 0 and Cin % 4 == 0 and lddu % 4 == 0 and ldx % 4 == 0, x_scale is not None,
                                  _wgrad_octets(x, du, N, Cin, lddu, ldx, du_off, x_off)),
                2.0 * M * N * ks * ks * Cin, x.element_size() * M * (N + Cin) + 4.0 * N * ks * ks * Cin):
        capi.check(capi.lib().ly_wgrad(ctypes.byref(P), capi.stream_ptr()), "ly_wgrad")


def _wgrad_params(*, M, H, W, N, du, lddu, x, ldx, Hin, Win, Cin, dw, lddw, ks=1, stride=1, pad=0, nchw=False, up2=False, du_off=0, x_off=0,
                  dw_off=0, dw_ts=None, dw_cs=1, n_valid=None, c_valid=None, x_scale=None, x_shift=None):
    def at(t, off):
        return ctypes.c_void_p(t.data_ptr() + t.element_size() * off)
    if du.dtype != x.dtype:
        raise capi.HipLibraryError(f"wgrad: du ({du.dtype}) and x ({x.dtype}) must share one storage dtype")
    if (x_scale is None) != (x_shift is None):
        raise ValueError("wgrad: x_scale and x_shift come together")
    if x_scale is not None and (x_scale.dtype != torch.float32 or x_shift.dtype != torch.float32 or x_scale.numel() < Cin or x_shift.numel() < Cin):
        raise ValueError("wgrad: x_scale / x_shift must be float32 vectors of at least Cin elements")
    ws = wgrad_workspace(x.device)
    return capi.LyWgradParams(M, H, W, N, at(du, du_off), lddu, at(x, x_off), ldx, Hin, Win, Cin, ks, stride, pad, int(nchw), int(up2),
                              at(dw, dw_off), lddw, capi.dtype_code(x), Cin if dw_ts is None else dw_ts, dw_cs, N if n_valid is None else n_valid,
                              Cin if c_valid is None else c_valid, _p(x_scale), _p(x_shift), _p(ws), ws.numel() if ws is not None else 0)


WGRAD_WS_FLOATS = 24 << 20
_WGRAD_WS = {}


def wgrad_workspace(device):
    if WGRAD_WS_FLOATS <= 0:
        return None
    ws = _WGRAD_WS.get(device)
    if ws is None:
        if torch.cuda.is_current_stream_capturing():
            return None
        ws = _WGRAD_WS[device] = torch.empty(WGRAD_WS_FLOATS, dtype=torch.float32, device=device)
    return ws


def _wgrad_groupable(q, dtype):
    return (q.get("ks", 1) == 1 and q.get("stride", 1) == 1 and q.get("pad", 0) == 0 and not q.get("nchw") and not q.get("up2")
            and q["N"] > 64 and q["N"] % 4 == 0 and q["Cin"] % 4 == 0 and q["lddu"] % 4 == 0 and q["ldx"] % 4 == 0
            and q["Hin"] == q["H"] and q["Win"] == q["W"] and q["x"].dtype == dtype)


class _WgradQueue:
    items = []
    notify = []
    task = -1


WGRAD_DEFER = True
WGRAD_GROUP_MAX = 4
WGRAD_DEFER_MAX_MACS = 4 << 30


def _wgrad_deferrable(q):
    return (WGRAD_DEFER and SINK is not None and q["x"].dtype == torch.bfloat16 and _wgrad_groupable(q, torch.bfloat16)
            and q["Cin"] > 64 and q["M"] * q["N"] * q["Cin"] <= WGRAD_DEFER_MAX_MACS and q.get("dw_off", 0) == 0 and SINK.is_target(q["dw"]) and _graph_task() >= 0)


def _wgrad_span(q):
    lo = q["dw"].data_ptr() + 4 * q.get("dw_off", 0)
    return lo, lo + 4 * q["N"] * q["lddw"]


def _wgrad_enqueue(q):
    task = _graph_task()
    if _WgradQueue.task != task:
        _WgradQueue.items, _WgradQueue.notify, _WgradQueue.task = [], [], task
        torch.autograd.Variable._execution_engine.queue_callback(wgrad_flush)
    lo, hi = _wgrad_span(q)
    if any(l2 < hi and lo < h2 for l2, h2 in map(_wgrad_span, _WgradQueue.items)):
        wgrad_flush(final=False)
    q["_versions"] = tuple(t._version for t in (q["du"], q["x"], q.get("x_scale"), q.get("x_shift")) if t is not None)
    _WgradQueue.items.append(q)
    if len(_WgradQueue.items) >= (2 if GRAD_LISTENERS else WGRAD_GROUP_MAX):
        wgrad_flush(final=False)


def wgrad_flush(final=True):
    items, _WgradQueue.items = _WgradQueue.items, []
    if final:
        _WgradQueue.task = -1
    for q in items:
        now = tuple(t._version for t in (q["du"], q["x"], q.get("x_scale"), q.get("x_shift")) if t is not None)
        if now != q.pop("_versions", now):
            raise RuntimeError("ops.wgrad: an operand of a deferred weight gradient was written in place before its launch (du / x / x_scale / "
                               "x_shift must stay untouched until the group leaves: see _wgrad_enqueue)")
    if len(items) == 1:
        wgrad(_now=True, **items[0])
    elif items:
        wgrad_group(items, _now=True)
    if _WgradQueue.notify:
        spans = [_wgrad_span(q) for q in _WgradQueue.items]
        waits = lambda ptr: any(lo <= ptr < hi for lo, hi in spans)
        ready = [prm for prm, ptr in _WgradQueue.notify if not waits(ptr)]
        _WgradQueue.notify = [(prm, ptr) for prm, ptr in _WgradQueue.notify if waits(ptr)]
        for prm in ready:
            for fn in GRAD_LISTENERS:
                fn(prm)


def wgrad_group(problems, _now=False):
    if not _now and all(_wgrad_deferrable(q) for q in problems):
        for q in problems:
            _wgrad_enqueue(q)
        return
    if not (2 <= len(problems) <= 4) or not all(_wgrad_groupable(q, problems[0]["x"].dtype) for q in problems):
        for q in problems:
            wgrad(_now=_now, **q)
        return
    arr = (capi.LyWgradParams * len(problems))(*[_wgrad_params(**q) for q in problems])
    x0 = problems[0]["x"]
    px = 128 if x0.dtype == torch.bfloat16 else 64
    anyp = any(q.get("x_scale") is not None for q in problems)
    gslab = wgrad_workspace(x0.device) is not None
    octs = gslab and all(_wgrad_octets(q["x"], q["du"], q["N"], q["Cin"], q["lddu"], q["ldx"], q.get("du_off", 0), q.get("x_off", 0)) for q in problems)
    with _Timed(f"ly_wgrad_tiled_group_kernel<{_tname(x0)}, 128, 128, {px}, true, {'true' if anyp else 'false'}, {'true' if gslab else 'false'}, "
                f"{'true' if octs else 'false'}>", sum(2.0 * q["M"] * q["N"] * q["Cin"] for q in problems),
                sum(x0.element_size() * q["M"] * (q["N"] + q["Cin"]) + 4.0 * q["N"] * q["Cin"] for q in problems)):
        capi.check(capi.lib().ly_wgrad_group(arr, len(problems), capi.stream_ptr()), "ly_wgrad_group")


def _wgrad_octets(x, du, n, cin, lddu, ldx, du_off=0, x_off=0):
    return (x.dtype == torch.bfloat16 and n % 8 == 0 and cin % 8 == 0 and lddu % 8 == 0 and ldx % 8 == 0
            and (du.data_ptr() + 2 * du_off) % 16 == 0 and (x.data_ptr() + 2 * x_off) % 16 == 0)


def wgrad_kernel_name(t, n, ktot, rows, tiled, pro=False, octets=False):
    r = "true" if rows else "false"
    if not tiled:
        return f"ly_wgrad_kernel<{t}, {r}>"
    px = 128 if t == "__bf16" else 64
    if n <= 64 and ktot <= 64:
        bn, bk = 64, 64
    elif n <= 32:
        bn, bk = 32, 128
    elif n <= 64:
        bn, bk = 64, 128
    else:
        bn, bk = 128, 128
    return f"ly_wgrad_tiled_kernel<{t}, {bn}, {bk}, {px}, {r}, {'true' if pro and rows else 'false'}, {'true' if octets else 'false'}>"


def sum_rows(t, out=None, accumulate=False):
    if t.dtype != torch.float32 or not t.is_contiguous():
        raise ValueError("sum_rows: contiguous float32 tensor expected")
    r = t.shape[0]
    c = t.numel() // r
    if out is None:
        out = torch.empty(t.shape[1:], dtype=torch.float32, device=t.device)
    capi.check(capi.lib().ly_sum_rows(_p(t), r, c, c, _p(out), int(accumulate), capi.stream_ptr()), "ly_sum_rows")
    return out


def up2_bwd(d, ldd, n, hs, ws, c):
    out = empty_nhwc(n, c, hs, ws, d)
    capi.check(capi.lib().ly_up2_bwd(_p(d), ldd, n, hs, ws, c, _p(out), c, capi.dtype_code(d), capi.stream_ptr()), "ly_up2_bwd")
    return out


def unpatch(g, n, ho, wo, c, ks, h, w):
    exact = (h == ho * ks and w == wo * ks)
    if not exact:
        raise NotImplementedError("patch-gather backward needs H, W divisible by the patch size")
    dx = empty_nhwc(n, c, h, w, g)
    capi.check(capi.lib().ly_unpatch(_p(g), n, ho, wo, c, ks, _p(dx), capi.dtype_code(g), capi.stream_ptr()), "ly_unpatch")
    return dx


def patch4_rows_u8(img, dtype):
    n, c, h, w = img.shape
    if img.dtype != torch.uint8 or not img.is_contiguous() or h % 4 or w % 4:
        raise ValueError("patch4_rows_u8: contiguous uint8 NCHW image with H, W multiples of 4 expected")
    rows = torch.empty((n * (h // 4) * (w // 4), 16 * c), dtype=dtype, device=img.device)
    capi.check(capi.lib().ly_patch4_rows_u8(_p(img), n, c, h, w, _p(rows), capi.dtype_code(rows), capi.stream_ptr()), "ly_patch4_rows_u8")
    return rows


def patch4_wgrad_u8_ok(img, du, n_out):
    n, c, h, w = img.shape
    ws = wgrad_workspace(img.device)
    return (img.dtype == torch.uint8 and img.is_contiguous() and c == 3 and h % 4 == 0 and w % 4 == 0 and du.dtype == torch.bfloat16
            and n_out % 8 == 0 and 8 <= n_out <= 64 and du.data_ptr() % 16 == 0 and ws is not None and ws.numel() >= 1536 * n_out * 48
            and n * (h // 4) * (w // 4) < (1 << 24))


def patch4_wgrad_u8(img, du, lddu, n_out, dw, scale):
    n, c, h, w = img.shape
    m = n * (h // 4) * (w // 4)
    ws = wgrad_workspace(img.device)
    with _Timed("ly_patch4_wgrad_u8_kernel", 2.0 * m * n_out * 48, 1.0 * n * c * h * w + 2.0 * m * n_out + 4.0 * n_out * 48):
        capi.check(capi.lib().ly_patch4_wgrad_u8(_p(img), n, c, h, w, _p(du), lddu, n_out, float(scale), _p(ws), ws.numel(), _p(dw), capi.dtype_code(du),
                                                 capi.stream_ptr()), "ly_patch4_wgrad_u8")


def coordatt_gate_bwd(dout, x, ldx, n, h, w, c, a_h, a_w, ldd=None):
    ldd = c if ldd is None else ldd
    dx = empty_nhwc(n, c, h, w, x)
    groups = 256 // (c // 4)
    slabs, bands = -(-w // (groups * 8)), -(-h // 8)
    ph = torch.empty((slabs, n * h * c), dtype=torch.float32, device=dout.device)
    pw = torch.empty((bands, n * w * c), dtype=torch.float32, device=dout.device)
    with _Timed(f"ly_coordatt_gate_bwd_kernel<{_tname(x)}>", 6.0 * n * h * w * c, 3.0 * x.element_size() * n * h * w * c):
        capi.check(capi.lib().ly_coordatt_gate_bwd(_p(dout), ldd, _p(x), ldx, n, h, w, c, _p(a_h), _p(a_w), _p(dx), c, _p(ph), _p(pw), bands, slabs,
                                                   capi.dtype_code(x), capi.stream_ptr()), "ly_coordatt_gate_bwd")
    da_h = (sum_rows(ph) if slabs > 1 else ph[0]).view(n, h, c)
    da_w = (sum_rows(pw) if bands > 1 else pw[0]).view(n, w, c)
    return dx, da_h, da_w


def pool_hw_bwd(gp, n, h, w, c, dtype=torch.float32, into=None):
    dx = into if into is not None else empty_nhwc(n, c, h, w, gp, dtype=dtype)
    capi.check(capi.lib().ly_pool_hw_bwd(_p(gp), n, h, w, c, _p(dx), c, 1 if into is not None else 0, capi.dtype_code(dx), capi.stream_ptr()),
               "ly_pool_hw_bwd")
    return dx


def maxpool_bwd(x, x_off, ldx, dy, dy_off, lddy, n, h, w, c, k, dx, dx_off, lddx):
    at = lambda t, off: ctypes.c_void_p(t.data_ptr() + t.element_size() * off)
    assert dy.dtype == torch.float32 and dx.dtype == torch.float32
    capi.check(capi.lib().ly_maxpool_bwd(at(x, x_off), ldx, at(dy, dy_off), lddy, n, h, w, c, k, at(dx, dx_off), lddx, capi.dtype_code(x),
                                         capi.stream_ptr()), "ly_maxpool_bwd")
```

Before: 7085 images/sec.

## Defer wgrad split-K combine into the next wgrad kernel's prologue

Split-K weight-gradient reductions no longer get their own combine kernel right after each wgrad launch. A pending-fold descriptor is carried forward and folded by the blocks of the next chained wgrad kernel (or flushed explicitly), which removes many small combine launches per backward pass. This needs overlap checks on dw spans, a larger workspace (slabs must double-buffer while a fold is pending), and Python-side chain state with flushes at the end of backward and before the patch4 wgrad. The risks are extra prologue work in the wgrad kernels, more LDS and register pressure, and correctness hazards if a flush is missed.

```diff
diff --git a/include/lead_yolo_hip.h b/include/lead_yolo_hip.h
--- a/include/lead_yolo_hip.h
+++ b/include/lead_yolo_hip.h
@@ -271,6 +271,25 @@
 } LyWgradParams;
 int ly_wgrad(const LyWgradParams* p, void* stream);
 int ly_wgrad_group(const LyWgradParams* arr, int n, void* stream);
+#define LY_WGRAD_PENDING_MAX 4
+typedef struct LyWgradFoldProblem {
+  float* dw; const float* slab;
+  int lddw, dw_ts, dw_cs, n_valid, c_valid, Cin, ktot;
+  int chunks, tiles_k, tiles, grp0;
+} LyWgradFoldProblem;
+enum { LY_WGRAD_PENDING_NONE = 0, LY_WGRAD_PENDING_TILED = 1, LY_WGRAD_PENDING_GROUP = 2, LY_WGRAD_PENDING_W3 = 3 };
+typedef struct LyWgradPending {
+  int kind;
+  int n;
+  int rls;
+  int BN, BK;
+  int groups;
+  int half;
+  LyWgradFoldProblem p[LY_WGRAD_PENDING_MAX];
+} LyWgradPending;
+int ly_wgrad_chained(const LyWgradParams* p, LyWgradPending* pend, void* stream);
+int ly_wgrad_group_chained(const LyWgradParams* arr, int n, LyWgradPending* pend, void* stream);
+int ly_wgrad_pending_flush(LyWgradPending* pend, void* stream);
 int ly_tune_wgrad3(int on);
 
 int ly_up2_bwd(const void* d , int ldd, int n_img, int Hs, int Ws, int C, void* out , int ldo, int dtype, void* stream);
diff --git a/lead-yolo_amd/csrc/ly_backward.hip b/lead-yolo_amd/csrc/ly_backward.hip
--- a/lead-yolo_amd/csrc/ly_backward.hip
+++ b/lead-yolo_amd/csrc/ly_backward.hip
@@ -784,31 +784,60 @@
   }
 }
 
-__device__ __forceinline__ void ly_wgrad_combine_body(const LyWgradParams& P, const float* __restrict__ slab, const int chunks, const int tiles_k,
-                                                      const int tiles, const int BN, const int BK, const long blk, const int rls) {
-  const long E = (long)tiles * BN * BK;
-  const long e = blk * 64 + (threadIdx.x & 63);
-  const int tile = (int)(e / (BN * BK));
-  const int rem = (int)(e - (long)tile * (BN * BK));
-  const int lr = rem / BK, lc = rem - lr * BK;
-  const int tk = tile % tiles_k, tn = tile / tiles_k;
-  const int row = tn * BN + lr, col = tk * BK + lc;
-  const int tap = col / P.Cin, cch = col - tap * P.Cin;
-  const bool live = e < E && row < P.n_valid && col < P.ks * P.ks * P.Cin && cch < P.c_valid;
-  ly_wgrad_fold(slab + e, E, chunks, rls, live, P.dw + (long)row * P.lddw + (long)tap * P.dw_ts + (long)cch * P.dw_cs);
-}
-__global__ __launch_bounds__(1024) void ly_wgrad_combine_kernel(const LyWgradParams P, const float* __restrict__ slab, const int chunks, const int tiles_k,
-                                                               const int tiles, const int BN, const int BK, const int rls) {
-  ly_wgrad_combine_body(P, slab, chunks, tiles_k, tiles, BN, BK, (long)blockIdx.x, rls);
-}
-static void wgrad_combine_launch(const LyWgradParams& P, const float* slab, long chunks, int tiles_k, long tiles, int BN, int BK, hipStream_t st) {
-  const long E = tiles * BN * BK;
-  const int rls = chunks <= 192 ? 4 : 16;
-  hipLaunchKernelGGL(ly_wgrad_combine_kernel, dim3((unsigned)((E + 63) / 64)), dim3(64 * rls), 0, st, P, slab, (int)chunks, tiles_k, (int)tiles, BN, BK, rls);
-}
+__global__ __launch_bounds__(1024) void ly_wgrad_combine_kernel(const LyWgradPending F) {
+  __shared__ float red[16 * 64];
+  ly_wgrad_fold_group(F, (int)blockIdx.x, red);
+}
+__global__ __launch_bounds__(1024) void ly_wgrad_combine_group_kernel(const LyWgradPending F) {
+  __shared__ float red[16 * 64];
+  ly_wgrad_fold_group(F, (int)blockIdx.x, red);
+}
+void ly_wgrad_pending_launch(const LyWgradPending& F, hipStream_t st) {
+  if (F.kind == LY_WGRAD_PENDING_W3) ly_wgrad3_fold_launch(F, st);
+  else if (F.kind == LY_WGRAD_PENDING_GROUP) hipLaunchKernelGGL(ly_wgrad_combine_group_kernel, dim3((unsigned)F.groups), dim3(64 * F.rls), 0, st, F);
+  else if (F.kind == LY_WGRAD_PENDING_TILED) hipLaunchKernelGGL(ly_wgrad_combine_kernel, dim3((unsigned)F.groups), dim3(64 * F.rls), 0, st, F);
+}
+extern "C" int ly_wgrad_pending_flush(LyWgradPending* pend, void* stream) {
+  LY_CHECK(pend, "wgrad_pending_flush: null descriptor");
+  if (pend->kind == LY_WGRAD_PENDING_NONE) return 0;
+  LY_CHECK(pend->kind <= LY_WGRAD_PENDING_W3 && pend->n >= 1 && pend->n <= LY_WGRAD_PENDING_MAX && (pend->rls == 4 || pend->rls == 16) && pend->groups > 0,
+           "wgrad_pending_flush: not a descriptor a chained launch left");
+  ly_wgrad_pending_launch(*pend, reinterpret_cast<hipStream_t>(stream));
+  pend->kind = LY_WGRAD_PENDING_NONE;
+  LY_LAUNCH_CHECK();
+  return 0;
+}
+static LyWgradFoldProblem wgrad_fold_problem(const LyWgradParams& P, const float* slab, long chunks, int tiles_k, long tiles, int grp0) {
+  LyWgradFoldProblem q;
+  q.dw = P.dw; q.slab = slab;
+  q.lddw = P.lddw; q.dw_ts = P.dw_ts; q.dw_cs = P.dw_cs; q.n_valid = P.n_valid; q.c_valid = P.c_valid; q.Cin = P.Cin; q.ktot = P.ks * P.ks * P.Cin;
+  q.chunks = (int)chunks; q.tiles_k = tiles_k; q.tiles = (int)tiles; q.grp0 = grp0;
+  return q;
+}
+static bool wgrad_pending_overlaps(const LyWgradPending& pend, const LyWgradParams& P) {
+  const float* lo = P.dw;
+  const float* hi = P.dw + (long)(P.n_valid - 1) * P.lddw + P.lddw;
+  for (int i = 0; i < (pend.kind != LY_WGRAD_PENDING_NONE ? pend.n : 0); ++i) {
+    const LyWgradFoldProblem& q = pend.p[i];
+    if (q.dw < hi && lo < q.dw + (long)q.n_valid * q.lddw) return true;
+  }
+  return false;
+}
+
+template <typename T, int BN, int BK, bool ROWS, bool PRO>
+constexpr bool ly_wgrad_tiled_carries() {
+  return ROWS && !(LyT<T>::BF && PRO && ((BN == 64 && BK == 64) || BN == 32)) && !(!LyT<T>::BF && BN == 128 && !PRO);
+}
+template <typename T, bool PRO, bool GSLAB, bool OCT>
+constexpr bool ly_wgrad_group_carries() { return GSLAB && !(LyT<T>::BF && PRO && !OCT); }
 
 template <typename T, int BN, int BK, int P, bool ROWS, bool PRO = false, bool OCT = false>
-__global__ __launch_bounds__(LY_THREADS) __attribute__((amdgpu_waves_per_eu(BN + BK > 160 ? 2 : 3))) void ly_wgrad_tiled_kernel(const LyWgradParams P_, const int tiles_k, const long chunk_px, float* const slab) {
+__global__ __launch_bounds__(LY_THREADS) __attribute__((amdgpu_waves_per_eu(BN + BK > 160 ? 2 : 3))) void ly_wgrad_tiled_kernel(const LyWgradParams P_, const int tiles_k, const long chunk_px, float* const slab, const LyWgradPending F) {
+  if constexpr (ly_wgrad_tiled_carries<T, BN, BK, ROWS, PRO>()) {
+    extern __shared__ f32x4 ly_smem4[];
+    if (F.kind != LY_WGRAD_PENDING_NONE)
+      ly_wgrad_fold_slice(F, (int)(blockIdx.y * gridDim.x + blockIdx.x), (int)(gridDim.x * gridDim.y), reinterpret_cast<float*>(ly_smem4));
+  }
   ly_wgrad_tiled_body<T, BN, BK, P, ROWS, PRO, 1, OCT>(P_, (int)blockIdx.x, (int)blockIdx.y, tiles_k, chunk_px, slab, (int)gridDim.x);
 }
 
@@ -818,11 +847,14 @@
   long chunk_px[LY_WGRAD_GROUP_MAX];
   float* slab[LY_WGRAD_GROUP_MAX];
   int tiles_k[LY_WGRAD_GROUP_MAX], tiles[LY_WGRAD_GROUP_MAX], blk0[LY_WGRAD_GROUP_MAX + 1];
-  int chunks[LY_WGRAD_GROUP_MAX], cblk0[LY_WGRAD_GROUP_MAX + 1];
   int n;
 };
 template <typename T, int BN, int BK, int P, bool ROWS, bool PRO = false, bool GSLAB = false, bool OCT = false>
-__global__ __launch_bounds__(LY_THREADS) __attribute__((amdgpu_waves_per_eu(BN + BK > 160 ? 2 : 3))) void ly_wgrad_tiled_group_kernel(const LyWgradGroupArgs G) {
+__global__ __launch_bounds__(LY_THREADS) __attribute__((amdgpu_waves_per_eu(BN + BK > 160 ? 2 : 3))) void ly_wgrad_tiled_group_kernel(const LyWgradGroupArgs G, const LyWgradPending F) {
+  if constexpr (ly_wgrad_group_carries<T, PRO, GSLAB, OCT>()) {
+    extern __shared__ f32x4 ly_smem4[];
+    if (F.kind != LY_WGRAD_PENDING_NONE) ly_wgrad_fold_slice(F, (int)blockIdx.x, (int)gridDim.x, reinterpret_cast<float*>(ly_smem4));
+  }
   const int bid = ly_xcd_remap((int)blockIdx.x, (int)gridDim.x);
   int g = 0;
 #pragma unroll
@@ -833,15 +865,6 @@
   const int tiles = G.tiles[g];
   ly_wgrad_tiled_body<T, BN, BK, P, ROWS, PRO, GSLAB ? 2 : 0, OCT>(G.p[g], local % tiles, local / tiles, G.tiles_k[g], G.chunk_px[g], GSLAB ? G.slab[g] : nullptr, tiles);
 }
-__global__ __launch_bounds__(1024) void ly_wgrad_combine_group_kernel(const LyWgradGroupArgs G, const int BN, const int BK, const int rls) {
-  int g = 0;
-#pragma unroll
-  for (int i = 1; i < LY_WGRAD_GROUP_MAX; ++i)
-    if (i < G.n && (int)blockIdx.x >= G.cblk0[i]) g = i;
-  g = __builtin_amdgcn_readfirstlane(g);
-  ly_wgrad_combine_body(G.p[g], G.slab[g], G.chunks[g], G.tiles_k[g], G.tiles[g], BN, BK, (long)((int)blockIdx.x - G.cblk0[g]), rls);
-}
-
 static long wg_target_blocks(bool group) {
 #ifdef LY_DEVEL
   static long t[2] = {0, 0};
@@ -868,7 +891,7 @@
 }
 
 template <typename T, int BN, int BK, int P>
-static int launch_wgrad_tiled(const LyWgradParams& Q, bool rows, hipStream_t st) {
+static int launch_wgrad_tiled(const LyWgradParams& Q, bool rows, LyWgradPending* pend, hipStream_t st) {
   const int Ktot = Q.ks * Q.ks * Q.Cin;
   const int tiles_n = (Q.N + BN - 1) / BN, tiles_k = (Ktot + BK - 1) / BK;
   const long tiles = (long)tiles_n * tiles_k;
@@ -882,11 +905,16 @@
   LY_CHECK(chunks < 65536, "wgrad: too many pixel chunks");
   const size_t lds = (LyT<T>::PL * P >= 128 ? 1 : 2) * (size_t)LyT<T>::PL * (P / 8) * (BN + BK + 16) * 16 + 2 * BK * sizeof(float);
   const dim3 grid((unsigned)tiles, (unsigned)chunks);
-  const long need = chunks * tiles * (long)(BN * BK);
-  float* const slab = (chunks > 1 && Q.ws && need <= Q.ws_floats) ? Q.ws : nullptr;
+  const bool pro = rows && Q.x_scale;
+  if (pend && !(!rows ? ly_wgrad_tiled_carries<T, BN, BK, false, false>() : pro ? ly_wgrad_tiled_carries<T, BN, BK, true, true>() : ly_wgrad_tiled_carries<T, BN, BK, true, false>())) {
+    LY_TRY(ly_wgrad_pending_flush(pend, st));
+    pend = nullptr;
+  }
+  LyWgradPlan plan;
+  LY_TRY(ly_wgrad_plan(Q, chunks > 1 ? chunks * tiles * (long)(BN * BK) : 0, pend, st, plan));
+  float* const slab = plan.slab;
 #define WG_TILED(ROWS_, PRO_, OCT_) \
-  ly_launch_lds<ly_wgrad_tiled_kernel<T, BN, BK, P, ROWS_, PRO_, OCT_>>(grid, dim3(LY_THREADS), lds, st, Q, tiles_k, chunk_px, slab)
-  const bool pro = rows && Q.x_scale;
+  ly_launch_lds<ly_wgrad_tiled_kernel<T, BN, BK, P, ROWS_, PRO_, OCT_>>(grid, dim3(LY_THREADS), lds, st, Q, tiles_k, chunk_px, slab, plan.carry)
   const auto launch = [&]() -> int {
     if constexpr (LyT<T>::BF) {
       if (wgrad_octets<T>(Q)) return !rows ? WG_TILED(false, false, true) : pro ? WG_TILED(true, true, true) : WG_TILED(true, false, true);
@@ -895,13 +923,23 @@
   };
 #undef WG_TILED
   LY_TRY(launch());
-  if (slab) wgrad_combine_launch(Q, slab, chunks, tiles_k, tiles, BN, BK, st);
+  LyWgradPending own{};
+  if (slab) {
+    own.kind = LY_WGRAD_PENDING_TILED;
+    own.n = 1;
+    own.rls = chunks <= 192 ? 4 : 16;
+    own.BN = BN;
+    own.BK = BK;
+    own.groups = (int)((tiles * BN * BK + 63) / 64);
+    own.p[0] = wgrad_fold_problem(Q, slab, chunks, tiles_k, tiles, 0);
+  }
+  ly_wgrad_leave(own, plan, pend, st);
   LY_LAUNCH_CHECK();
   return 0;
 }
 
 template <typename T>
-static int wgrad_dispatch(const LyWgradParams& P, void* stream);
+static int wgrad_dispatch(const LyWgradParams& P, LyWgradPending* pend, void* stream);
 static int g_ly_wgrad3 = 1;
 extern "C" int ly_tune_wgrad3(int on) {
   const int was = g_ly_wgrad3;
@@ -912,7 +950,13 @@
 extern "C" int ly_wgrad(const LyWgradParams* p, void* stream) {
   LY_CHECK(p, "wgrad: null params");
   LY_CHECK_DTYPE(p->dtype, "wgrad");
-  return p->dtype == LY_BF16 ? wgrad_dispatch<__bf16>(*p, stream) : wgrad_dispatch<float>(*p, stream);
+  return p->dtype == LY_BF16 ? wgrad_dispatch<__bf16>(*p, nullptr, stream) : wgrad_dispatch<float>(*p, nullptr, stream);
+}
+extern "C" int ly_wgrad_chained(const LyWgradParams* p, LyWgradPending* pend, void* stream) {
+  LY_CHECK(p && pend, "wgrad_chained: null params / descriptor");
+  LY_CHECK_DTYPE(p->dtype, "wgrad_chained");
+  if (wgrad_pending_overlaps(*pend, *p)) LY_TRY(ly_wgrad_pending_flush(pend, stream));
+  return p->dtype == LY_BF16 ? wgrad_dispatch<__bf16>(*p, pend, stream) : wgrad_dispatch<float>(*p, pend, stream);
 }
 
 template <typename T>
@@ -926,7 +970,7 @@
 }
 
 template <typename T>
-static int wgrad_group_launch(const LyWgradParams* arr, int n, hipStream_t st) {
+static int wgrad_group_launch(const LyWgradParams* arr, int n, LyWgradPending* pend, hipStream_t st) {
   constexpr int PX = LyT<T>::BF ? 128 : 64, BN = 128, BK = 128;
   LyWgradGroupArgs G;
   long tiles_total = 0;
@@ -938,6 +982,7 @@
   }
   G.n = n;
   G.blk0[0] = 0;
+  int nchunks[LY_WGRAD_GROUP_MAX];
   for (int g = 0; g < n; ++g) {
     long chunks = (wg_target_blocks(true) + tiles_total - 1) / tiles_total;
     const long max_chunks = (arr[g].M + 511) / 512;
@@ -947,24 +992,25 @@
     chunk_px = (chunk_px + PX - 1) / PX * PX;
     chunks = (arr[g].M + chunk_px - 1) / chunk_px;
     G.chunk_px[g] = chunk_px;
-    G.chunks[g] = (int)chunks;
+    nchunks[g] = (int)chunks;
     G.blk0[g + 1] = G.blk0[g] + (int)(chunks * G.tiles[g]);
   }
-  for (int g = n; g < LY_WGRAD_GROUP_MAX; ++g) { G.tiles_k[g] = G.tiles[g] = 1; G.chunk_px[g] = PX; G.blk0[g + 1] = G.blk0[n]; G.p[g] = arr[0]; G.chunks[g] = 0; G.slab[g] = nullptr; }
-  bool gslab = arr[0].ws != nullptr && (long)G.blk0[n] * (BN * BK) <= arr[0].ws_floats;
-  G.cblk0[0] = 0;
-  for (int g = 0; g < n; ++g) {
-    G.slab[g] = gslab ? arr[0].ws + (long)G.blk0[g] * (BN * BK) : nullptr;
-    G.cblk0[g + 1] = G.cblk0[g] + (int)(((long)G.tiles[g] * BN * BK + 63) / 64);
-  }
-  for (int g = n; g < LY_WGRAD_GROUP_MAX; ++g) G.cblk0[g + 1] = G.cblk0[n];
-  const size_t lds = (LyT<T>::PL * PX >= 128 ? 1 : 2) * (size_t)LyT<T>::PL * (PX / 8) * (BN + BK + 16) * 16 + 2 * BK * sizeof(float);
+  for (int g = n; g < LY_WGRAD_GROUP_MAX; ++g) { G.tiles_k[g] = G.tiles[g] = 1; G.chunk_px[g] = PX; G.blk0[g + 1] = G.blk0[n]; G.p[g] = arr[0]; G.slab[g] = nullptr; }
   bool any_pro = false;
   for (int g = 0; g < n; ++g) any_pro = any_pro || arr[g].x_scale != nullptr;
   bool oct = true;
   for (int g = 0; g < n; ++g) oct = oct && wgrad_octets<T>(arr[g]);
+  if (pend && LyT<T>::BF && any_pro && !oct) {
+    LY_TRY(ly_wgrad_pending_flush(pend, st));
+    pend = nullptr;
+  }
+  LyWgradPlan plan;
+  LY_TRY(ly_wgrad_plan(arr[0], (long)G.blk0[n] * (BN * BK), pend, st, plan));
+  const bool gslab = plan.slab != nullptr;
+  for (int g = 0; g < n; ++g) G.slab[g] = gslab ? plan.slab + (long)G.blk0[g] * (BN * BK) : nullptr;
+  const size_t lds = (LyT<T>::PL * PX >= 128 ? 1 : 2) * (size_t)LyT<T>::PL * (PX / 8) * (BN + BK + 16) * 16 + 2 * BK * sizeof(float);
 #define WG_GROUP(PRO_, GSLAB_, OCT_) \
-  ly_launch_lds<ly_wgrad_tiled_group_kernel<T, BN, BK, PX, true, PRO_, GSLAB_, OCT_>>(dim3((unsigned)G.blk0[n]), dim3(LY_THREADS), lds, st, G)
+  ly_launch_lds<ly_wgrad_tiled_group_kernel<T, BN, BK, PX, true, PRO_, GSLAB_, OCT_>>(dim3((unsigned)G.blk0[n]), dim3(LY_THREADS), lds, st, G, plan.carry)
   const auto launch = [&]() -> int {
     if (!gslab) return any_pro ? WG_GROUP(true, false, false) : WG_GROUP(false, false, false);
     if constexpr (LyT<T>::BF) {
@@ -974,17 +1020,26 @@
   };
 #undef WG_GROUP
   LY_TRY(launch());
+  LyWgradPending own{};
   if (gslab) {
     int cmax = 0;
-    for (int g = 0; g < n; ++g) cmax = G.chunks[g] > cmax ? G.chunks[g] : cmax;
-    const int rls = cmax <= 64 ? 4 : 16;
-    hipLaunchKernelGGL(ly_wgrad_combine_group_kernel, dim3((unsigned)G.cblk0[n]), dim3(64 * rls), 0, st, G, BN, BK, rls);
-    LY_LAUNCH_CHECK();
-  }
-  return 0;
-}
-
-extern "C" int ly_wgrad_group(const LyWgradParams* arr, int n, void* stream) {
+    for (int g = 0; g < n; ++g) cmax = nchunks[g] > cmax ? nchunks[g] : cmax;
+    own.kind = LY_WGRAD_PENDING_GROUP;
+    own.n = n;
+    own.rls = cmax <= 64 ? 4 : 16;
+    own.BN = BN;
+    own.BK = BK;
+    for (int g = 0; g < n; ++g) {
+      own.p[g] = wgrad_fold_problem(arr[g], G.slab[g], nchunks[g], G.tiles_k[g], G.tiles[g], own.groups);
+      own.groups += (int)(((long)G.tiles[g] * BN * BK + 63) / 64);
+    }
+  }
+  ly_wgrad_leave(own, plan, pend, st);
+  LY_LAUNCH_CHECK();
+  return 0;
+}
+
+static int wgrad_group_any(const LyWgradParams* arr, int n, LyWgradPending* pend, void* stream) {
   LY_CHECK(arr && n > 0, "wgrad_group: bad arguments");
   bool same = n >= 2 && n <= LY_WGRAD_GROUP_MAX;
   for (int g = 0; g < n && same; ++g) {
@@ -993,17 +1048,27 @@
   }
   if (!same) {
     for (int g = 0; g < n; ++g) {
-      const int rc = ly_wgrad(arr + g, stream);
+      const int rc = pend ? ly_wgrad_chained(arr + g, pend, stream) : ly_wgrad(arr + g, stream);
       if (rc) return rc;
     }
     return 0;
   }
   hipStream_t st = reinterpret_cast<hipStream_t>(stream);
-  return arr[0].dtype == LY_BF16 ? wgrad_group_launch<__bf16>(arr, n, st) : wgrad_group_launch<float>(arr, n, st);
+  if (pend) {
+    bool overlap = false;
+    for (int g = 0; g < n; ++g) overlap = overlap || wgrad_pending_overlaps(*pend, arr[g]);
+    if (overlap) LY_TRY(ly_wgrad_pending_flush(pend, stream));
+  }
+  return arr[0].dtype == LY_BF16 ? wgrad_group_launch<__bf16>(arr, n, pend, st) : wgrad_group_launch<float>(arr, n, pend, st);
+}
+extern "C" int ly_wgrad_group(const LyWgradParams* arr, int n, void* stream) { return wgrad_group_any(arr, n, nullptr, stream); }
+extern "C" int ly_wgrad_group_chained(const LyWgradParams* arr, int n, LyWgradPending* pend, void* stream) {
+  LY_CHECK(pend, "wgrad_group_chained: null descriptor");
+  return wgrad_group_any(arr, n, pend, stream);
 }
 
 template <typename T>
-static int wgrad_dispatch(const LyWgradParams& P, void* stream) {
+static int wgrad_dispatch(const LyWgradParams& P, LyWgradPending* pend, void* stream) {
   LY_CHECK(P.du && P.x && P.dw, "wgrad: null pointer");
   LY_CHECK(P.M > 0 && P.H > 0 && P.W > 0 && P.N > 0 && P.Cin > 0 && P.ks > 0 && P.stride > 0, "wgrad: bad sizes");
   LY_CHECK(P.M < (1L << 24), "wgrad: M=%ld pixels exceeds the 2^24 limit of the fast index path", P.M);
@@ -1017,15 +1082,16 @@
   const bool tiled_ok = !P.nchw && (P.N & 3) == 0 && (P.Cin & 3) == 0 && (P.lddu & 3) == 0 && (P.ldx & 3) == 0 && ((uintptr_t)P.du & (4 * sizeof(T) - 1)) == 0 &&
                         ((uintptr_t)P.x & (4 * sizeof(T) - 1)) == 0;
   if (P.x_scale) LY_CHECK(rows && tiled_ok, "wgrad: the x prologue is built for plain-row 1x1 problems with vector-friendly widths");
-  if (g_ly_wgrad3 && ly_wgrad3_ok(P)) return ly_wgrad3_launch(P, reinterpret_cast<hipStream_t>(stream));
+  if (g_ly_wgrad3 && ly_wgrad3_ok(P)) return ly_wgrad3_launch(P, pend, reinterpret_cast<hipStream_t>(stream));
   if (!P.nchw && (P.N & 3) == 0 && (P.Cin & 3) == 0 && (P.lddu & 3) == 0 && (P.ldx & 3) == 0 && ((uintptr_t)P.du & (4 * sizeof(T) - 1)) == 0 && ((uintptr_t)P.x & (4 * sizeof(T) - 1)) == 0) {
     hipStream_t st2 = reinterpret_cast<hipStream_t>(stream);
     constexpr int PX = LyT<T>::BF ? 128 : 64;
-    if (P.N <= 64 && Ktot <= 64) return launch_wgrad_tiled<T, 64, 64, PX>(P, rows, st2);
-    if (P.N <= 32) return launch_wgrad_tiled<T, 32, 128, PX>(P, rows, st2);
-    if (P.N <= 64) return launch_wgrad_tiled<T, 64, 128, PX>(P, rows, st2);
-    return launch_wgrad_tiled<T, 128, 128, PX>(P, rows, st2);
-  }
+    if (P.N <= 64 && Ktot <= 64) return launch_wgrad_tiled<T, 64, 64, PX>(P, rows, pend, st2);
+    if (P.N <= 32) return launch_wgrad_tiled<T, 32, 128, PX>(P, rows, pend, st2);
+    if (P.N <= 64) return launch_wgrad_tiled<T, 64, 128, PX>(P, rows, pend, st2);
+    return launch_wgrad_tiled<T, 128, 128, PX>(P, rows, pend, st2);
+  }
+  if (pend) LY_TRY(ly_wgrad_pending_flush(pend, stream));
   const int tiles_n = (P.N + 63) / 64, tiles_k = (Ktot + 63) / 64;
   const long tiles = (long)tiles_n * tiles_k;
   long chunks = (2048 + tiles - 1) / tiles;
diff --git a/lead-yolo_amd/csrc/ly_wgrad.hpp b/lead-yolo_amd/csrc/ly_wgrad.hpp
--- a/lead-yolo_amd/csrc/ly_wgrad.hpp
+++ b/lead-yolo_amd/csrc/ly_wgrad.hpp
@@ -3,38 +3,183 @@
 #include "ly_params.h"
 
 bool ly_wgrad3_ok(const LyWgradParams& P);
-int ly_wgrad3_launch(const LyWgradParams& P, hipStream_t st);
+int ly_wgrad3_launch(const LyWgradParams& P, LyWgradPending* pend, hipStream_t st);
+void ly_wgrad3_fold_launch(const LyWgradPending& F, hipStream_t st);
 
-__device__ __forceinline__ void ly_wgrad_fold(const float* __restrict__ p, const long E, const int chunks, const int rls, const bool live, float* const d) {
-  __shared__ float red[16 * 64];
-  const int rl = threadIdx.x >> 6;
+__device__ __forceinline__ float ly_wgrad_fold_lane(const float* __restrict__ p, const long E, const int chunks, const int rls, const int rl) {
   float a0 = 0.f, a1 = 0.f, a2 = 0.f, a3 = 0.f;
-  if (live) {
-    int c = rl;
-    for (; c + 7 * rls < chunks; c += 8 * rls) {
-      float v[8];
+  int c = rl;
+  for (; c + 7 * rls < chunks; c += 8 * rls) {
+    float v[8];
 #pragma unroll
-      for (int k = 0; k < 8; ++k) v[k] = p[(long)(c + rls * k) * E];
-      __builtin_amdgcn_sched_barrier(0);
-      a0 += v[0]; a1 += v[1]; a2 += v[2]; a3 += v[3];
-      a0 += v[4]; a1 += v[5]; a2 += v[6]; a3 += v[7];
-    }
-    for (; c + 3 * rls < chunks; c += 4 * rls) {
-      float v[4];
+    for (int k = 0; k < 8; ++k) v[k] = p[(long)(c + rls * k) * E];
+    __builtin_amdgcn_sched_barrier(0);
+    a0 += v[0]; a1 += v[1]; a2 += v[2]; a3 += v[3];
+    a0 += v[4]; a1 += v[5]; a2 += v[6]; a3 += v[7];
+  }
+  for (; c + 3 * rls < chunks; c += 4 * rls) {
+    float v[4];
 #pragma unroll
-      for (int k = 0; k < 4; ++k) v[k] = p[(long)(c + rls * k) * E];
-      __builtin_amdgcn_sched_barrier(0);
-      a0 += v[0]; a1 += v[1]; a2 += v[2]; a3 += v[3];
-    }
-    if (c < chunks) a0 += p[(long)c * E];
-    if (c + rls < chunks) a1 += p[(long)(c + rls) * E];
-    if (c + 2 * rls < chunks) a2 += p[(long)(c + 2 * rls) * E];
+    for (int k = 0; k < 4; ++k) v[k] = p[(long)(c + rls * k) * E];
+    __builtin_amdgcn_sched_barrier(0);
+    a0 += v[0]; a1 += v[1]; a2 += v[2]; a3 += v[3];
   }
-  red[threadIdx.x] = (a0 + a1) + (a2 + a3);
+  if (c < chunks) a0 += p[(long)c * E];
+  if (c + rls < chunks) a1 += p[(long)(c + rls) * E];
+  if (c + 2 * rls < chunks) a2 += p[(long)(c + 2 * rls) * E];
+  return (a0 + a1) + (a2 + a3);
+}
+__device__ __forceinline__ void ly_wgrad_fold(const float* __restrict__ p, const long E, const int chunks, const int rls, const bool live, float* const d,
+                                              float* const red ) {
+  red[threadIdx.x] = live ? ly_wgrad_fold_lane(p, E, chunks, rls, threadIdx.x >> 6) : 0.f;
   __syncthreads();
-  if (rl == 0 && live) {
+  if (threadIdx.x < 64 && live) {
     float s = 0.f;
     for (int i = 0; i < rls; ++i) s += red[64 * i + threadIdx.x];
     *d += s;
   }
 }
+
+struct LyWgradFoldTarget {
+  const float* p;
+  float* d;
+  long E;
+  int chunks;
+  bool live;
+};
+__device__ __forceinline__ LyWgradFoldTarget ly_wgrad_fold_decode(const LyWgradPending& F, const int grp, const int col64) {
+  int g = 0;
+#pragma unroll
+  for (int i = 1; i < LY_WGRAD_PENDING_MAX; ++i)
+    if (i < F.n && grp >= F.p[i].grp0) g = i;
+  g = __builtin_amdgcn_readfirstlane(g);
+  const LyWgradFoldProblem& Q = F.p[g];
+  const int tile_elems = F.BN * F.BK;
+  const long E = (long)Q.tiles * tile_elems;
+  const long e = (long)(grp - Q.grp0) * 64 + col64;
+  const int tile = (int)(e / tile_elems);
+  const int rem = (int)(e - (long)tile * tile_elems);
+  const int lr = rem / F.BK, lc = rem - lr * F.BK;
+  int row, tap, cch;
+  bool live = e < E;
+  if (F.kind == LY_WGRAD_PENDING_W3) {
+    const int cn = tile % Q.tiles_k, cc = tile / Q.tiles_k;
+    const int ct = lc >> 4;
+    row = cn * F.BN + lr;
+    tap = ct >> 1;
+    cch = cc * 32 + (ct & 1) * 16 + (lc & 15);
+  } else {
+    const int tk = tile % Q.tiles_k, tn = tile / Q.tiles_k;
+    const int col = tk * F.BK + lc;
+    row = tn * F.BN + lr;
+    tap = col / Q.Cin;
+    cch = col - tap * Q.Cin;
+    live = live && col < Q.ktot;
+  }
+  live = live && row < Q.n_valid && cch < Q.c_valid;
+  LyWgradFoldTarget t;
+  t.p = Q.slab + (live ? e : 0);
+  t.d = Q.dw + (live ? (long)row * Q.lddw + (long)tap * Q.dw_ts + (long)cch * Q.dw_cs : 0);
+  t.E = E;
+  t.chunks = Q.chunks;
+  t.live = live;
+  return t;
+}
+__device__ __forceinline__ void ly_wgrad_fold_group(const LyWgradPending& F, const int grp, float* const red) {
+  const LyWgradFoldTarget t = ly_wgrad_fold_decode(F, grp, threadIdx.x & 63);
+  ly_wgrad_fold(t.p, t.E, t.chunks, F.rls, t.live, t.d, red);
+}
+
+__device__ __forceinline__ void ly_wgrad_fold_lanes4(const float* __restrict__ p, const long E, const int chunks, const int rls, const int rl0, const int step,
+                                                     float (&out)[4]) {
+  float a[4][4];
+#pragma unroll
+  for (int i = 0; i < 4; ++i)
+#pragma unroll
+    for (int j = 0; j < 4; ++j) a[i][j] = 0.f;
+  int k = 0;
+  for (; rl0 + 3 * step + (k + 7) * rls < chunks; k += 8) {
+    float v[4][8];
+#pragma unroll
+    for (int j = 0; j < 8; ++j)
+#pragma unroll
+      for (int i = 0; i < 4; ++i) v[i][j] = p[(long)(rl0 + i * step + (k + j) * rls) * E];
+    __builtin_amdgcn_sched_barrier(0);
+#pragma unroll
+    for (int j = 0; j < 8; ++j)
+#pragma unroll
+      for (int i = 0; i < 4; ++i) a[i][j & 3] += v[i][j];
+  }
+  if (rl0 + k * rls < chunks) {
+    float v[4][8];
+#pragma unroll
+    for (int j = 0; j < 8; ++j)
+#pragma unroll
+      for (int i = 0; i < 4; ++i) {
+        const int c = rl0 + i * step + (k + j) * rls;
+        v[i][j] = p[(long)(c < chunks ? c : 0) * E];
+      }
+    __builtin_amdgcn_sched_barrier(0);
+#pragma unroll
+    for (int j = 0; j < 8; ++j)
+#pragma unroll
+      for (int i = 0; i < 4; ++i) a[i][j & 3] = rl0 + i * step + (k + j) * rls < chunks ? a[i][j & 3] + v[i][j] : a[i][j & 3];
+  }
+#pragma unroll
+  for (int i = 0; i < 4; ++i) out[i] = (a[i][0] + a[i][1]) + (a[i][2] + a[i][3]);
+}
+
+__device__ __forceinline__ void ly_wgrad_fold_slice(const LyWgradPending& F, const int block, const int nblocks, float* const red) {
+  const int wave = __builtin_amdgcn_readfirstlane(threadIdx.x >> 6), col = threadIdx.x & 63;
+  const bool per_wave = F.rls == 4;
+  for (int grp = per_wave ? 4 * block + wave : block; grp < F.groups; grp += per_wave ? 4 * nblocks : nblocks) {
+    const LyWgradFoldTarget t = ly_wgrad_fold_decode(F, grp, col);
+    const float d0 = *(t.live ? t.d : t.p);
+    float r[4];
+    ly_wgrad_fold_lanes4(t.p, t.E, t.chunks, F.rls, per_wave ? 0 : wave, per_wave ? 1 : 4, r);
+    if (per_wave) {
+      if (t.live) *t.d = d0 + (((0.f + r[0]) + r[1]) + r[2] + r[3]);
+    } else {
+#pragma unroll
+      for (int i = 0; i < 4; ++i) red[64 * (wave + 4 * i) + col] = t.live ? r[i] : 0.f;
+      __syncthreads();
+      if (wave == 0 && t.live) {
+        float s = 0.f;
+        for (int i = 0; i < 16; ++i) s += red[64 * i + col];
+        *t.d = d0 + s;
+      }
+      __syncthreads();
+    }
+  }
+}
+
+void ly_wgrad_pending_launch(const LyWgradPending& F, hipStream_t st);
+
+struct LyWgradPlan {
+  float* slab;
+  int half;
+  LyWgradPending carry;
+};
+inline int ly_wgrad_plan(const LyWgradParams& P, const long need, LyWgradPending*& pend, hipStream_t st, LyWgradPlan& plan) {
+  plan.slab = nullptr;
+  plan.half = 0;
+  plan.carry = LyWgradPending{};
+  if (pend) {
+    const long half_floats = P.ws ? (P.ws_floats / 2) & ~63L : 0;
+    if (need <= half_floats) {
+      plan.carry = *pend;
+      plan.half = pend->kind != LY_WGRAD_PENDING_NONE ? 1 - pend->half : 0;
+      plan.slab = need ? P.ws + plan.half * half_floats : nullptr;
+      return 0;
+    }
+    LY_TRY(ly_wgrad_pending_flush(pend, st));
+    pend = nullptr;
+  }
+  plan.slab = (need && P.ws && need <= P.ws_floats) ? P.ws : nullptr;
+  return 0;
+}
+inline void ly_wgrad_leave(LyWgradPending own, const LyWgradPlan& plan, LyWgradPending* pend, hipStream_t st) {
+  own.half = plan.half;
+  if (pend) *pend = own;
+  else ly_wgrad_pending_launch(own, st);
+}
diff --git a/lead-yolo_amd/csrc/ly_wgrad3.hip b/lead-yolo_amd/csrc/ly_wgrad3.hip
--- a/lead-yolo_amd/csrc/ly_wgrad3.hip
+++ b/lead-yolo_amd/csrc/ly_wgrad3.hip
@@ -19,8 +19,10 @@
 __global__ __launch_bounds__(LY_THREADS) __attribute__((amdgpu_waves_per_eu(4))) void ly_wgrad3_kernel(const LyWgradParams P, const int tiles_x,
                                                                                                         const int tiles_y, const int n_n,
                                                                                                         const int n_c, const int tchunk,
-                                                                                                        const int total_tiles, float* __restrict__ const slab) {
+                                                                                                        const int total_tiles, float* __restrict__ const slab,
+                                                                                                        const LyWgradPending F) {
   __shared__ __attribute__((aligned(16))) char w3_lds[W3_DU_BYTES + W3_X_BYTES];
+  if (F.kind != LY_WGRAD_PENDING_NONE) ly_wgrad_fold_slice(F, (int)blockIdx.x, (int)gridDim.x, reinterpret_cast<float*>(w3_lds));
   char* const ds = w3_lds;
   char* const xs = w3_lds + W3_DU_BYTES;
   const int tid = threadIdx.x, lane = tid & 63;
@@ -167,19 +169,12 @@
   }
 }
 
-__global__ __launch_bounds__(1024) void ly_wgrad3_combine_kernel(const LyWgradParams P, const float* __restrict__ slab, const int chunks, const int n_n,
-                                                                const int n_c, const int rls) {
-  const long E = (long)n_c * n_n * (W3_BN * 288);
-  const long e = (long)blockIdx.x * 64 + (threadIdx.x & 63);
-  const int combo = (int)(e / (W3_BN * 288));
-  const int rem = (int)(e - (long)combo * (W3_BN * 288));
-  const int row = rem / 288, col = rem - row * 288;
-  const int cn = combo % n_n, cc = combo / n_n;
-  const int ct = col >> 4, li = col & 15;
-  const int orow = cn * W3_BN + row;
-  const int cch = cc * W3_CK + (ct & 1) * 16 + li;
-  const bool live = e < E && orow < P.n_valid && cch < P.c_valid;
-  ly_wgrad_fold(slab + e, E, chunks, rls, live, P.dw + (long)orow * P.lddw + (long)(ct >> 1) * P.dw_ts + (long)cch * P.dw_cs);
+__global__ __launch_bounds__(1024) void ly_wgrad3_combine_kernel(const LyWgradPending F) {
+  __shared__ float red[16 * 64];
+  ly_wgrad_fold_group(F, (int)blockIdx.x, red);
+}
+void ly_wgrad3_fold_launch(const LyWgradPending& F, hipStream_t st) {
+  hipLaunchKernelGGL(ly_wgrad3_combine_kernel, dim3((unsigned)F.groups), dim3(64 * F.rls), 0, st, F);
 }
 
 bool ly_wgrad3_ok(const LyWgradParams& P) {
@@ -188,7 +183,7 @@
          (reinterpret_cast<uintptr_t>(P.x) & 15) == 0;
 }
 
-int ly_wgrad3_launch(const LyWgradParams& P, hipStream_t st) {
+int ly_wgrad3_launch(const LyWgradParams& P, LyWgradPending* pend, hipStream_t st) {
   const int tiles_x = (P.W + 7) / 8, tiles_y = (P.H + 7) / 8;
   const long n_img = P.M / ((long)P.H * P.W);
   const long total = n_img * tiles_x * tiles_y;
@@ -208,14 +203,24 @@
   const long tchunk = (total + chunks - 1) / chunks;
   chunks = (total + tchunk - 1) / tchunk;
   const long need = chunks * n_n * n_c * (long)(W3_BN * 288);
-  float* slab = (P.ws && need <= P.ws_floats && !force_atomic) ? P.ws : nullptr;
+  LyWgradParams Pw = P;
+  if (force_atomic) Pw.ws = nullptr;
+  LyWgradPlan plan;
+  LY_TRY(ly_wgrad_plan(Pw, need, pend, st, plan));
+  float* const slab = plan.slab;
   hipLaunchKernelGGL(ly_wgrad3_kernel, dim3((unsigned)(chunks * n_n * n_c)), dim3(LY_THREADS), 0, st, P, tiles_x, tiles_y, n_n, n_c, (int)tchunk,
-                     (int)total, slab);
+                     (int)total, slab, plan.carry);
+  LyWgradPending own{};
   if (slab) {
-    const long E = (long)n_n * n_c * (W3_BN * 288);
-    const int rls = chunks <= 192 ? 4 : 16;
-    hipLaunchKernelGGL(ly_wgrad3_combine_kernel, dim3((unsigned)((E + 63) / 64)), dim3(64 * rls), 0, st, P, slab, (int)chunks, n_n, n_c, rls);
-  }
+    own.kind = LY_WGRAD_PENDING_W3;
+    own.n = 1;
+    own.rls = chunks <= 192 ? 4 : 16;
+    own.BN = W3_BN;
+    own.BK = 288;
+    own.groups = (int)(((long)n_n * n_c * (W3_BN * 288) + 63) / 64);
+    own.p[0] = LyWgradFoldProblem{P.dw, slab, P.lddw, P.dw_ts, P.dw_cs, P.n_valid, P.c_valid, P.Cin, 9 * P.Cin, (int)chunks, n_n, n_n * n_c, 0};
+  }
+  ly_wgrad_leave(own, plan, pend, st);
   LY_LAUNCH_CHECK();
   return 0;
 }
diff --git a/lead-yolo_amd/ops.py b/lead-yolo_amd/ops.py
--- a/lead-yolo_amd/ops.py
+++ b/lead-yolo_amd/ops.py
@@ -626,6 +626,7 @@
 def small_grads_reset():
     _SmallGrads.pending, _SmallGrads.task, _SmallGrads.announced, _SmallGrads.nodes = [], -1, set(), {}
     _WgradQueue.items, _WgradQueue.notify, _WgradQueue.task = [], [], -1
+    _wgrad_pending_drop()
 
 
 def small_grad_scratch(target, param):
@@ -1055,7 +1056,7 @@
                                   (not nchw) and N % 4 == 0 and Cin % 4 == 0 and lddu % 4 == 0 and ldx % 4 == 0, x_scale is not None,
                                   _wgrad_octets(x, du, N, Cin, lddu, ldx, du_off, x_off)),
                 2.0 * M * N * ks * ks * Cin, x.element_size() * M * (N + Cin) + 4.0 * N * ks * ks * Cin):
-        capi.check(capi.lib().ly_wgrad(ctypes.byref(P), capi.stream_ptr()), "ly_wgrad")
+        _wgrad_call([q], "ly_wgrad", ctypes.byref(P))
 
 
 def _wgrad_params(*, M, H, W, N, du, lddu, x, ldx, Hin, Win, Cin, dw, lddw, ks=1, stride=1, pad=0, nchw=False, up2=False, du_off=0, x_off=0,
@@ -1074,7 +1075,7 @@
                               Cin if c_valid is None else c_valid, _p(x_scale), _p(x_shift), _p(ws), ws.numel() if ws is not None else 0)
 
 
-WGRAD_WS_FLOATS = 24 << 20
+WGRAD_WS_FLOATS = 32 << 20
 _WGRAD_WS = {}
 
 
@@ -1101,6 +1102,50 @@
     task = -1
 
 
+class _WgradChain:
+    pend = {}
+    spans = {}
+    final = False
+
+
+def _wgrad_pass():
+    task = _graph_task()
+    if _WgradQueue.task != task:
+        _WgradQueue.items, _WgradQueue.notify, _WgradQueue.task = [], [], task
+        _wgrad_pending_drop()
+        torch.autograd.Variable._execution_engine.queue_callback(wgrad_flush)
+
+
+def _wgrad_pending_drop():
+    for pend in _WgradChain.pend.values():
+        pend.kind = 0
+    _WgradChain.spans = {}
+
+
+def wgrad_pending_flush(device=None):
+    for dev, pend in _WgradChain.pend.items():
+        if pend.kind and (device is None or dev == device):
+            with torch.cuda.device(dev):
+                capi.check(capi.lib().ly_wgrad_pending_flush(ctypes.byref(pend), capi.stream_ptr()), "ly_wgrad_pending_flush")
+            _WgradChain.spans[dev] = []
+
+
+def _wgrad_call(problems, entry, *args):
+    dev = problems[0]["x"].device
+    if (GRAD_LISTENERS or SINK is None or not all(SINK.is_target(q["dw"]) for q in problems) or wgrad_workspace(dev) is None
+            or not (_WgradChain.final or _graph_task() >= 0)):
+        wgrad_pending_flush(dev)
+        return capi.check(getattr(capi.lib(), entry)(*args, capi.stream_ptr()), entry)
+    if not _WgradChain.final:
+        _wgrad_pass()
+    pend = _WgradChain.pend.setdefault(dev, capi.LyWgradPending())
+    spans = [_wgrad_span(q) for q in problems]
+    if any(l2 < hi and lo < h2 for lo, hi in spans for l2, h2 in _WgradChain.spans.get(dev, ())):
+        wgrad_pending_flush(dev)
+    capi.check(getattr(capi.lib(), entry + "_chained")(*args, ctypes.byref(pend), capi.stream_ptr()), entry + "_chained")
+    _WgradChain.spans[dev] = spans if pend.kind else []
+
+
 WGRAD_DEFER = True
 WGRAD_GROUP_MAX = 4
 WGRAD_DEFER_MAX_MACS = 4 << 30
@@ -1117,10 +1162,7 @@
 
 
 def _wgrad_enqueue(q):
-    task = _graph_task()
-    if _WgradQueue.task != task:
-        _WgradQueue.items, _WgradQueue.notify, _WgradQueue.task = [], [], task
-        torch.autograd.Variable._execution_engine.queue_callback(wgrad_flush)
+    _wgrad_pass()
     lo, hi = _wgrad_span(q)
     if any(l2 < hi and lo < h2 for l2, h2 in map(_wgrad_span, _WgradQueue.items)):
         wgrad_flush(final=False)
@@ -1134,6 +1176,25 @@
     items, _WgradQueue.items = _WgradQueue.items, []
     if final:
         _WgradQueue.task = -1
+        _WgradChain.final = True
+    try:
+        _wgrad_flush_items(items)
+        if final:
+            wgrad_pending_flush()
+    finally:
+        if final:
+            _WgradChain.final = False
+    if _WgradQueue.notify:
+        spans = [_wgrad_span(q) for q in _WgradQueue.items]
+        waits = lambda ptr: any(lo <= ptr < hi for lo, hi in spans)
+        ready = [prm for prm, ptr in _WgradQueue.notify if not waits(ptr)]
+        _WgradQueue.notify = [(prm, ptr) for prm, ptr in _WgradQueue.notify if waits(ptr)]
+        for prm in ready:
+            for fn in GRAD_LISTENERS:
+                fn(prm)
+
+
+def _wgrad_flush_items(items):
     for q in items:
         now = tuple(t._version for t in (q["du"], q["x"], q.get("x_scale"), q.get("x_shift")) if t is not None)
         if now != q.pop("_versions", now):
@@ -1143,14 +1204,6 @@
         wgrad(_now=True, **items[0])
     elif items:
         wgrad_group(items, _now=True)
-    if _WgradQueue.notify:
-        spans = [_wgrad_span(q) for q in _WgradQueue.items]
-        waits = lambda ptr: any(lo <= ptr < hi for lo, hi in spans)
-        ready = [prm for prm, ptr in _WgradQueue.notify if not waits(ptr)]
-        _WgradQueue.notify = [(prm, ptr) for prm, ptr in _WgradQueue.notify if waits(ptr)]
-        for prm in ready:
-            for fn in GRAD_LISTENERS:
-                fn(prm)
 
 
 def wgrad_group(problems, _now=False):
@@ -1171,7 +1224,7 @@
     with _Timed(f"ly_wgrad_tiled_group_kernel<{_tname(x0)}, 128, 128, {px}, true, {'true' if anyp else 'false'}, {'true' if gslab else 'false'}, "
                 f"{'true' if octs else 'false'}>", sum(2.0 * q["M"] * q["N"] * q["Cin"] for q in problems),
                 sum(x0.element_size() * q["M"] * (q["N"] + q["Cin"]) + 4.0 * q["N"] * q["Cin"] for q in problems)):
-        capi.check(capi.lib().ly_wgrad_group(arr, len(problems), capi.stream_ptr()), "ly_wgrad_group")
+        _wgrad_call(problems, "ly_wgrad_group", arr, len(problems))
 
 
 def _wgrad_octets(x, du, n, cin, lddu, ldx, du_off=0, x_off=0):
@@ -1242,6 +1295,7 @@
     n, c, h, w = img.shape
     m = n * (h // 4) * (w // 4)
     ws = wgrad_workspace(img.device)
+    wgrad_pending_flush(img.device)
     with _Timed("ly_patch4_wgrad_u8_kernel", 2.0 * m * n_out * 48, 1.0 * n * c * h * w + 2.0 * m * n_out + 4.0 * n_out * 48):
         capi.check(capi.lib().ly_patch4_wgrad_u8(_p(img), n, c, h, w, _p(du), lddu, n_out, float(scale), _p(ws), ws.numel(), _p(dw), capi.dtype_code(du),
                                                  capi.stream_ptr()), "ly_patch4_wgrad_u8")
```

Measured after the change: 7118 images/sec (median of 6 runs). Within noise of the previous version (+0.5%).
